# AlexandreDubray/consistent-viterbi

Measured on AMD Instinct MI355X. Metric: trellis cells/s (N*T*batch), N=256 T=512 batch=65536, higher is better.
Workload: dtype f64

## Files before the change

consistent-viterbi_amd/csrc/cviterbi.cpp:

```cpp
#include <hip/hip_runtime.h>

#include <algorithm>
#include <atomic>
#include <charconv>
#include <chrono>
#include <cmath>
#include <cstdarg>
#include <cstdio>
#include <cstdlib>
#include <cstring>
#include <memory>
#include <functional>
#include <limits>
#include <mutex>
#include <numeric>
#include <string>
#include <thread>
#include <type_traits>
#include <vector>

#include "../../include/cviterbi.h"
#include "batchplan.hpp"
#include "csp.hpp"
#include "hostscan.hpp"
// ... 60 lines not shown
    if (p) {
      (void)hipFree(p);
      g_dev_cur -= (int64_t)bytes;
    }
    p = nullptr;
    bytes = 0;
  }
  cv_status ensure(size_t n) {
    if (n <= bytes && p) return CV_OK;
    release();
    if (n == 0) n = 16;
    hipError_t e = hipMalloc(&p, n);
    if (e != hipSuccess) {
      p = nullptr;
      (void)hipGetLastError();
      return set_err(CV_ENOMEM, "hipMalloc(%zu) failed: %s", n, hipGetErrorString(e));
    }
    bytes = n;
    const int64_t cur = g_dev_cur += (int64_t)n;
    int64_t pk = g_dev_peak.load();
    while (cur > pk && !g_dev_peak.compare_exchange_weak(pk, cur)) {
    }
    return CV_OK;
  }
  template <typename T>
  T* as() const {
    return static_cast<T*>(p);
  }
};

cv_status upload(DevBuf& buf, const void* src, size_t bytes) {
  cv_status st = buf.ensure(bytes);
  if (st != CV_OK) return st;
  HIP_TRY(hipMemcpy(buf.p, src, bytes, hipMemcpyHostToDevice));
  return CV_OK;
}

constexpr uint64_t kDefaultWorkspace = 8ull << 30;
constexpr uint64_t kDefaultWorkspaceT64 = 64ull << 30;
constexpr size_t kMaxTimedEvents = 1 << 16;

}

struct PinnedHost {
  void* p = nullptr;
  size_t cap = 0;
  PinnedHost() = default;
  PinnedHost(const PinnedHost&) = delete;
  PinnedHost& operator=(const PinnedHost&) = delete;
  ~PinnedHost() { release(); }
  void release() {
    if (p) (void)hipHostFree(p);
    p = nullptr;
    cap = 0;
  }
  bool ensure(size_t bytes) {
    if (cap >= bytes && p) return true;
    if (p) (void)hipHostFree(p);
    p = nullptr;
    cap = 0;
    const size_t want = std::max<size_t>(bytes, 4096);
    if (hipHostMalloc(&p, want, hipHostMallocDefault) != hipSuccess) {
      (void)hipGetLastError();
      return false;
    }
    cap = want;
    return true;
  }
  template <typename T>
  T* as() const { return static_cast<T*>(p); }
};

struct OrderStage {
  int32_t* p[2] = {nullptr, nullptr};
  size_t cap[2] = {0, 0};
  hipEvent_t ev[2] = {nullptr, nullptr};
  bool pending[2] = {false, false};
  int slot = 0;
  OrderStage() = default;
  OrderStage(const OrderStage&) = delete;
  OrderStage& operator=(const OrderStage&) = delete;
  ~OrderStage() {
    for (int k = 0; k < 2; ++k) {
      if (pending[k]) (void)hipEventSynchronize(ev[k]);
      if (p[k]) (void)hipHostFree(p[k]);
      if (ev[k]) (void)hipEventDestroy(ev[k]);
    }
  }
  int32_t* acquire(size_t n) {
    const int k = slot;
    if (pending[k]) {
      if (hipEventSynchronize(ev[k]) != hipSuccess) return nullptr;
      pending[k] = false;
    }
    if (!ev[k] && hipEventCreateWithFlags(&ev[k], hipEventDisableTiming) != hipSuccess) return nullptr;
    if (cap[k] < n) {
      if (p[k]) (void)hipHostFree(p[k]);
      p[k] = nullptr;
      cap[k] = 0;
      const size_t want = std::max<size_t>(n, 4096);
      if (hipHostMalloc((void**)&p[k], want * 4, hipHostMallocDefault) != hipSuccess) return nullptr;
      cap[k] = want;
    }
    return p[k];
  }
  hipError_t release(hipStream_t stream) {
    const hipError_t e = hipEventRecord(ev[slot], stream);
    pending[slot] = e == hipSuccess;
    slot ^= 1;
    return e;
  }
};

struct cv_hmm {
  int N = 0, D = 0;
  std::vector<int64_t> bdims;
  int64_t V = 0;
  std::vector<double> pi, a, b;
  int device = 0;
  int cus = 0;
  hipStream_t stream = nullptr;
  hipStream_t bt_stream = nullptr;
  std::mutex mu;
  cvk::Tuning tuning;

  int np = 0;
  DevBuf t_aimg, t_pi, t_et, t_at, t_arm;
  int npw = 0;
  DevBuf w_arm, w_pi, w_et, w_at;
  DevBuf t_aimg_T, t_pi0;
  bool f64_ready = false;
  DevBuf d_pi64, d_a64, d_et64;
  DevBuf d_at64;

  int np64 = 0;
  bool t64_ready = false;
  DevBuf q_a, q_at, q_pi, q_et;
  DevBuf q_at32;
  bool t64_nonpos = false;
  int nonpos_cache = -1;
  double arc_max = -1.0;
  double cert_rho_cap = 0.0;
  DevBuf t64_stats;
  PinnedHost t64_stats_pin;
  bool t64_lo_off = false;
  int fx_state = -1;
  DevBuf fx_aimg, fx_pi, fx_et, fx_at;
  double fx_gain = 0.0;
  DevBuf fx_cert, fx_idx, fx_obs2, fx_path2, fx_score2, fx_status2;
  PinnedHost fx_cert_pin;
  std::vector<int64_t> fx_idx_host;
  bool fx_pinned = false;
  int64_t fx_last[4] = {0, 0, 0, 0};
  DevBuf q_pi0;
  bool g32_ready = false;
  DevBuf d_pi32, d_a32, d_et32;
  DevBuf d_at32;
  int pnp = 0;
  DevBuf p_pi, p_a, p_at, p_et, p_dump;
  DevBuf ps_rows, ps_order, st_gamma;
  DevBuf ps_kshift;
  PinnedHost sm_pin;
  OrderStage ps_pin;
  DevBuf kb_bp, kb_last, kb_order, kb_end, st_count;
  OrderStage kb_pin;
  DevBuf ws_main, ws_last, ws_order;
  struct SideWs {
    DevBuf main, last, order, idx, obs2, path2, res2;
    std::vector<int32_t> order_host;
    OrderStage order_pin;
    hipEvent_t ws_done = nullptr;
    bool ws_rec = false;
    std::vector<int64_t> idx_host;
    std::vector<hipEvent_t> ev;
    hipStream_t stream = nullptr;
    hipStream_t hi = nullptr;
    hipEvent_t start = nullptr, done = nullptr, after = nullptr;
  } side;
  DevBuf st_off, st_obs, st_path, st_score, st_status, st_forced;
  DevBuf st_emis;
  DevBuf cs_ranges, cs_delta, cs_g, cs_mu, cs_start, cs_zero, cs_queue;
  DevBuf cs_wrows;
  DevBuf cs_comp, cs_words;
  DevBuf cs_flag;
  DevBuf cs_seg;
  DevBuf rs_rows, rs_rowbase, rs_resume, rs_start, rs_off2, rs_ridx, rs_slot, rs_obs2, rs_frc2, rs_path2;
  DevBuf rs_srows, rs_srowbase, rs_cert;
  hipEvent_t rs_ev = nullptr;
  std::vector<int32_t> order_host;
  OrderStage order_pin;
  hipEvent_t ws_done = nullptr;
  bool ws_rec = false;
  std::vector<float> host_dl, host_mu;
  std::vector<int64_t> sort_pos;
  std::vector<hipEvent_t> ev;
  int64_t last_launches = 0;
  size_t last_ev_base = 0;
  bool acc_on = false, acc_overflow = false;
  size_t acc_used = 0;
  int32_t last_kernel = 0;
  int32_t last_np = 0;
  int32_t last_mt = -1;
  uint64_t last_explored = 0;
  int64_t last_traced = 0;
  int64_t last_chain[9] = {0, 0, 0, 0, 0, 0, 0, 0, 0};
  struct ChainBufs {
    DevBuf off, obs, path, res, cert, ebin, q, ends, gid, gpath;
    DevBuf first, rpsi, rows, small, rpath, soff, sobs, spath, sres, sinit, slast, spsi;
  } chainb;
  hipStream_t chain_stream = nullptr;
  std::vector<hipEvent_t> part_ev;
  std::vector<hipEvent_t> chunk_ev;
  std::vector<hipEvent_t> emis_ev;
  hipStream_t copy_stream = nullptr;
  PinnedHost chain_pin;
  PinnedHost chain_gpin;
  PinnedHost chain_obs_pin, chain_ring[2];
  hipEvent_t ring_ev[2] = {nullptr, nullptr};

  ~cv_hmm() {
    for (auto e : ring_ev)
      if (e) (void)hipEventDestroy(e);
    for (auto e : ev) (void)hipEventDestroy(e);
    for (auto e : side.ev) (void)hipEventDestroy(e);
    if (side.start) (void)hipEventDestroy(side.start);
    if (side.done) (void)hipEventDestroy(side.done);
    if (side.after) (void)hipEventDestroy(side.after);
    if (side.stream) (void)hipStreamDestroy(side.stream);
    if (side.hi) (void)hipStreamDestroy(side.hi);
    if (rs_ev) (void)hipEventDestroy(rs_ev);
    if (ws_done) (void)hipEventDestroy(ws_done);
    if (side.ws_done) (void)hipEventDestroy(side.ws_done);
    if (stream) (void)hipStreamDestroy(stream);
    if (bt_stream) (void)hipStreamDestroy(bt_stream);
    for (auto e : chunk_ev) (void)hipEventDestroy(e);
    for (auto e : emis_ev) (void)hipEventDestroy(e);
    for (auto e : part_ev) (void)hipEventDestroy(e);
    if (copy_stream) (void)hipStreamDestroy(copy_stream);
    if (chain_stream) (void)hipStreamDestroy(chain_stream);
  }
};

namespace {

uint64_t free_device_bytes(uint64_t held) {
  size_t fr = 0, tot = 0;
  if (hipMemGetInfo(&fr, &tot) != hipSuccess) {
    (void)hipGetLastError();
    return 0;
  }
  return (uint64_t)fr + held;
}

uint64_t default_workspace_cap(uint64_t held, uint64_t base) {
  const uint64_t avail = free_device_bytes(held);
  if (avail == 0) return base;
  return std::max<uint64_t>(std::min<uint64_t>(base, avail / 4 * 3), 256ull << 20);
}

cv_status set_device(cv_hmm* h) {
  int n = 0;
  if (hipGetDeviceCount(&n) != hipSuccess || n <= 0) {
    (void)hipGetLastError();
    return set_err(CV_EDEVICE, "no HIP device available");
  }
  if (h->device < 0 || h->device >= n) return set_err(CV_EDEVICE, "device %d out of range (%d devices)", h->device, n);
  HIP_TRY(hipSetDevice(h->device));
  if (!h->cus) HIP_TRY(hipDeviceGetAttribute(&h->cus, hipDeviceAttributeMultiprocessorCount, h->device));
  if (!h->stream) HIP_TRY(hipStreamCreateWithFlags(&h->stream, hipStreamNonBlocking));
  if (!h->bt_stream) HIP_TRY(hipStreamCreateWithFlags(&h->bt_stream, hipStreamNonBlocking));
  return CV_OK;
}

float f32(double x) { return (float)x; }

cv_status ensure_trellis_tables(cv_hmm* h) {
  const int np = cvk::trellis_padded_states(h->N);
  if (!np) return set_err(CV_EUNSUPPORTED, "trellis kernel covers 1 <= N <= 256 (N=%d)", h->N);
  if (h->np == np) return CV_OK;
  const int N = h->N;
  const int64_t V = h->V;
  const int R = np / 8;
  const float NI = -INFINITY;
  auto A = [&](int i, int j) -> float { return (i < N && j < N) ? f32(h->a[(size_t)i * N + j]) : NI; };
  std::vector<float> img((size_t)np * np);
  for (int w = 0; w < np / 16; ++w)
    for (int q = 0; q < R / 2; ++q)
      for (int lane = 0; lane < 64; ++lane) {
        const int rg = lane & 7, cp = lane >> 3, j0 = 16 * w + 2 * cp, r0 = rg * R + 2 * q;
        float* dst = &img[(((size_t)w * (R / 2) + q) * 64 + lane) * 4];
        dst[0] = A(r0, j0);
        dst[1] = A(r0, j0 + 1);
        dst[2] = A(r0 + 1, j0);
        dst[3] = A(r0 + 1, j0 + 1);
      }
  std::vector<float> pi(np, NI), at((size_t)np * np, NI), arm((size_t)np * np, NI), et((size_t)V * np, NI);
  for (int j = 0; j < N; ++j) pi[j] = f32(h->pi[j]);
  for (int i = 0; i < N; ++i)
    for (int j = 0; j < N; ++j) at[(size_t)j * np + i] = arm[(size_t)i * np + j] = f32(h->a[(size_t)i * N + j]);
  for (int j = 0; j < N; ++j)
    for (int64_t o = 0; o < V; ++o) et[(size_t)o * np + j] = f32(h->b[(size_t)j * V + o]);
  cv_status st;
  if ((st = upload(h->t_aimg, img.data(), img.size() * 4)) != CV_OK) return st;
  {
    auto AT = [&](int i, int j) -> float { return A(j, i); };
    std::vector<float> imgT((size_t)np * np);
// ... 1129 lines not shown
    if (err == hipSuccess) err = cvkb::launch_kbest_walk(g, stream);
    if (err != hipSuccess) return set_err(CV_EDEVICE, "K-best select / walk launch failed: %s", hipGetErrorString(err));
    HIP_TRY(hipEventRecord(b1, stream));
    h->last_launches = (int64_t)ci + 1;
  }
  return end_call(h, false, nev, stream);
}

cv_opts default_opts() {
  cv_opts o;
  cv_opts_init(&o);
  return o;
}

struct HostBatch {
  cv_hmm* h;
  int64_t nseq;
  const int64_t* offsets;
  const int32_t* obs;
  hipStream_t stream;
  int64_t base = 0, total = 0;
  hipError_t err = hipSuccess;

  size_t plane() const { return (size_t)std::max<int64_t>(total, 1); }

  cv_status stage(cv_opts& o, size_t planes, size_t width, bool check_obs = false, bool forced_host = true) {
    cv_status st = check_batch(nseq, offsets);
    if (st != CV_OK) return st;
    base = offsets[0], total = offsets[nseq];
    const int32_t* ob = check_obs ? obs : nullptr;
    const int32_t* fr = forced_host ? o.forced : nullptr;
    const int64_t V = h->V, N = h->N;
    int64_t k;
    if (ob && (k = first_bad(base, total, [&](int64_t i) { return ob[i] < 0 || ob[i] >= V; })) >= 0)
      return set_err(CV_EINVAL, "obs[%lld] = %d out of range [0,%lld)", (long long)k, ob[k], (long long)V);
    if (fr && (k = first_bad(base, total, [&](int64_t i) { return fr[i] < -1 || fr[i] >= N; })) >= 0)
      return set_err(CV_EINVAL, "forced[%lld] = %d out of range [-1,%d)", (long long)k, fr[k], h->N);
    if ((st = h->st_off.ensure((size_t)(nseq + 1) * 8)) != CV_OK) return st;
    if (obs && (st = h->st_obs.ensure(plane() * 4)) != CV_OK) return st;
    if (planes && (st = h->st_path.ensure(plane() * planes * 4)) != CV_OK) return st;
    if ((st = h->st_score.ensure((size_t)nseq * width * 8)) != CV_OK) return st;
    if ((st = h->st_status.ensure((size_t)nseq)) != CV_OK) return st;
    if (fr && (st = h->st_forced.ensure(plane() * 4)) != CV_OK) return st;
    HIP_TRY(hipMemcpyAsync(h->st_off.p, offsets, (size_t)(nseq + 1) * 8, hipMemcpyHostToDevice, stream));
    const size_t n = (size_t)(total - base) * 4;
    if (obs && n) HIP_TRY(hipMemcpyAsync(h->st_obs.as<int32_t>() + base, obs + base, n, hipMemcpyHostToDevice, stream));
    if (fr && n) HIP_TRY(hipMemcpyAsync(h->st_forced.as<int32_t>() + base, fr + base, n, hipMemcpyHostToDevice, stream));
    if (fr) o.forced = h->st_forced.as<int32_t>();
    return CV_OK;
  }
  cv_status stage_emis(const double* emis, int64_t ld, EmisSrc* src) {
    const int64_t N = h->N, rows = total - base;
    cv_status st = h->st_emis.ensure((size_t)std::max<int64_t>(rows, 1) * N * 8);
    if (st != CV_OK) return st;
    if (rows > 0)
      HIP_TRY(hipMemcpy2DAsync(h->st_emis.p, (size_t)N * 8, emis + base * ld, (size_t)ld * 8, (size_t)N * 8,
                               (size_t)rows, hipMemcpyHostToDevice, stream));
    *src = EmisSrc{reinterpret_cast<const double*>(reinterpret_cast<uintptr_t>(h->st_emis.p) -
                                                   (uintptr_t)base * (uintptr_t)N * 8),
                   N};
    return CV_OK;
  }
  cv_status fail(cv_status st) const {
    (void)hipStreamSynchronize(stream);
    return st;
  }
  template <typename T>
  void fetch_elems(T* out, const DevBuf& buf, size_t width = 1, size_t r = 0) {
    const size_t at = (r * (size_t)total + (size_t)base) * width, n = (size_t)(total - base) * width * sizeof(T);
    if (err == hipSuccess && n) err = hipMemcpyAsync(out + at, buf.as<T>() + at, n, hipMemcpyDeviceToHost, stream);
  }
  template <typename T>
  void fetch_seqs(T* out, const DevBuf& buf, size_t width = 1) {
    if (err == hipSuccess) err = hipMemcpyAsync(out, buf.p, (size_t)nseq * width * sizeof(T), hipMemcpyDeviceToHost, stream);
  }
  cv_status finish() {
    if (err == hipSuccess) err = hipStreamSynchronize(stream);
    return err == hipSuccess ? CV_OK : set_err(CV_EDEVICE, "copying the results back failed: %s", hipGetErrorString(err));
  }
};

}

extern "C" {

CV_API const char* cv_last_error(void) { return g_err.c_str(); }
CV_API const char* cv_version(void) { return "cviterbi 0.1.0 (gfx950)"; }
CV_API int32_t cv_abi_version(void) { return CV_ABI_VERSION; }
CV_API cv_status cv_device_memory(int64_t* current_bytes, int64_t* peak_bytes) {
  if (current_bytes) *current_bytes = g_dev_cur.load();
  if (peak_bytes) *peak_bytes = g_dev_peak.load();
  return CV_OK;
}
CV_API int32_t cv_device_count(void) {
  int n = 0;
  if (hipGetDeviceCount(&n) != hipSuccess) {
    (void)hipGetLastError();
    return 0;
  }
  return n;
}

CV_API void cv_opts_init(cv_opts* o) {
  if (!o) return;
  std::memset(o, 0, sizeof *o);
  o->dtype = CV_DTYPE_F64;
  o->assoc = CV_ASSOC_VITERBI;
  o->kernel = CV_KERNEL_AUTO;
  o->rescore_f64 = 1;
}

CV_API cv_status cv_hmm_create(const cv_hmm_desc* d, cv_hmm** out) {
  if (!d || !out) return set_err(CV_EINVAL, "null argument");
  if (d->ndims <= 0 || !d->bdims) return set_err(CV_EINVAL, "ndims/bdims required");
  std::vector<int64_t> bd(d->bdims, d->bdims + d->ndims);
  return make_hmm(d->nstates, bd, d->pi, d->a, d->b, d->device, out);
}

CV_API cv_status cv_hmm_from_json(const char* path, int32_t device, cv_hmm** out) {
  if (!path || !out) return set_err(CV_EINVAL, "null argument");
  std::string text, err;
  if (!cvh::read_file(path, text)) return set_err(CV_EIO, "cannot read %s", path);
  cvh::HmmJson j;
  if (!cvh::parse_hmm_json(text, j, err)) return set_err(CV_EPARSE, "%s", err.c_str());
  return make_hmm(j.nstates, j.bdims, j.pi.data(), j.a.data(), j.b.data(), device, out);
}

CV_API cv_status cv_hmm_write_json(const cv_hmm* h, const char* path) {
  if (!h || !path) return set_err(CV_EINVAL, "null argument");
  const std::string s = cvh::format_hmm_json(h->N, h->bdims, h->pi.data(), h->a.data(), h->b.data());
  FILE* f = fopen(path, "wb");
  if (!f) return set_err(CV_EIO, "cannot write %s", path);
  const size_t n = fwrite(s.data(), 1, s.size(), f);
  fclose(f);
  if (n != s.size()) return set_err(CV_EIO, "short write to %s", path);
  return CV_OK;
}

CV_API void cv_hmm_destroy(cv_hmm* h) {
  if (!h) return;
  int n = 0;
  if (hipGetDeviceCount(&n) == hipSuccess && h->device >= 0 && h->device < n) (void)hipSetDevice(h->device);
  delete h;
}

CV_API cv_status cv_hmm_set_tuning(cv_hmm* h, const char* key, int64_t value) {
  if (!h || !key) return set_err(CV_EINVAL, "bad argument");
  std::lock_guard<std::mutex> lk(h->mu);
  if (!cvk::tuning_set(h->tuning, key, value)) return set_err(CV_EINVAL, "unknown tuning key '%s' or value out of range", key);
  if (std::strcmp(key, "t64_nonpos") == 0) {
    h->nonpos_cache = -1;
    h->t64_ready = false;
    h->fx_state = -1;
  }
  return CV_OK;
}
CV_API cv_status cv_hmm_release_workspaces(cv_hmm* h) {
  if (!h) return set_err(CV_EINVAL, "null handle");
  CV_LOCK(h);
  cv_status st = set_device(h);
  if (st != CV_OK) return st;
  for (hipStream_t s : {h->stream, h->bt_stream, h->side.stream, h->side.hi, h->copy_stream, h->chain_stream})
    if (s) HIP_TRY(hipStreamSynchronize(s));
  if (h->ws_rec) HIP_TRY(hipEventSynchronize(h->ws_done));
  if (h->side.ws_rec) HIP_TRY(hipEventSynchronize(h->side.ws_done));
  for (DevBuf* b : {&h->ws_main, &h->ws_last, &h->ws_order, &h->side.main, &h->side.last, &h->side.order,
                    &h->side.idx, &h->side.obs2, &h->side.path2, &h->side.res2, &h->st_off, &h->st_obs, &h->st_path,
                    &h->st_score, &h->st_status, &h->st_forced, &h->cs_ranges, &h->cs_delta, &h->cs_g, &h->cs_mu,
                    &h->cs_start, &h->cs_zero, &h->cs_queue, &h->cs_wrows, &h->cs_comp, &h->cs_words, &h->cs_flag,
                    &h->cs_seg, &h->rs_rows, &h->rs_rowbase, &h->rs_resume, &h->rs_start, &h->rs_off2, &h->rs_ridx,
                    &h->rs_slot, &h->rs_obs2, &h->rs_frc2, &h->rs_path2, &h->rs_srows, &h->rs_srowbase, &h->rs_cert,
                    &h->chainb.off, &h->chainb.obs, &h->chainb.path, &h->chainb.res, &h->chainb.cert, &h->chainb.ebin,
                    &h->chainb.q, &h->chainb.ends, &h->chainb.gid, &h->chainb.gpath, &h->chainb.first,
                    &h->chainb.rpsi, &h->chainb.rows, &h->chainb.small, &h->chainb.rpath, &h->chainb.soff,
                    &h->chainb.sobs, &h->chainb.spath, &h->chainb.sres, &h->chainb.sinit, &h->chainb.slast,
                    &h->chainb.spsi, &h->ps_rows,
                    &h->ps_order, &h->ps_kshift, &h->st_gamma, &h->kb_bp, &h->kb_last, &h->kb_order, &h->kb_end, &h->st_count,
                    &h->st_emis, &h->fx_cert, &h->fx_idx, &h->fx_obs2, &h->fx_path2, &h->fx_score2, &h->fx_status2})
    b->release();
  h->fx_cert_pin.release();
  h->sm_pin.release();
  h->ws_rec = false;
  h->side.ws_rec = false;
  h->chain_pin.release();
  h->chain_gpin.release();
  h->chain_obs_pin.release();
  h->chain_ring[0].release();
  h->chain_ring[1].release();
  return CV_OK;
}
CV_API cv_status cv_hmm_get_tuning(const cv_hmm* h, const char* key, int64_t* value) {
  if (!h || !key || !value) return set_err(CV_EINVAL, "bad argument");
  std::lock_guard<std::mutex> lk(const_cast<cv_hmm*>(h)->mu);
  if (!cvk::tuning_get(h->tuning, key, value)) return set_err(CV_EINVAL, "unknown tuning key '%s'", key);
  return CV_OK;
}
CV_API const char* cv_tuning_key(int32_t i) { return cvk::tuning_key(i); }
CV_API int32_t cv_hmm_nstates(const cv_hmm* h) { return h ? h->N : -1; }
CV_API int64_t cv_hmm_nobs(const cv_hmm* h) { return h ? h->V : -1; }
CV_API int32_t cv_hmm_ndims(const cv_hmm* h) { return h ? h->D : -1; }
CV_API cv_status cv_hmm_bdims(const cv_hmm* h, int64_t* out) {
  if (!h || !out) return set_err(CV_EINVAL, "null argument");
  std::copy(h->bdims.begin(), h->bdims.end(), out);
  return CV_OK;
}

CV_API cv_status cv_obs_flatten(const cv_hmm* h, const int64_t* value, int64_t* flat) {
  if (!h || !value || !flat) return set_err(CV_EINVAL, "null argument");
  int64_t f = 0;
  for (int d = 0; d < h->D; ++d) {
    if (value[d] < 0 || value[d] >= h->bdims[d])
      return set_err(CV_EINVAL, "observation component %d = %lld out of range [0,%lld)", d, (long long)value[d],
                     (long long)h->bdims[d]);
    f = f * h->bdims[d] + value[d];
  }
  *flat = f;
  return CV_OK;
}

static bool lookup_ok(const cv_hmm* h, int32_t s, int64_t o) {
  return h && s >= 0 && s < h->N && o >= 0 && o < h->V;
}

CV_API double cv_hmm_init_prob(const cv_hmm* h, int32_t state, int64_t obs) {
  if (!lookup_ok(h, state, obs)) return NAN;
  return h->pi[state] + h->b[(size_t)state * h->V + obs];
}
CV_API cv_status cv_hmm_init_probs(const cv_hmm* h, int64_t obs, double* out) {
  if (!lookup_ok(h, 0, obs) || !out) return set_err(CV_EINVAL, "bad argument");
  for (int s = 0; s < h->N; ++s) out[s] = h->pi[s] + h->b[(size_t)s * h->V + obs];
  return CV_OK;
}
CV_API double cv_hmm_transition_prob(const cv_hmm* h, int32_t from, int32_t to, int64_t obs) {
  if (!lookup_ok(h, to, obs) || from < 0 || from >= h->N) return NAN;
  return h->a[(size_t)from * h->N + to] + h->b[(size_t)to * h->V + obs];
}
CV_API cv_status cv_hmm_transitions_to(const cv_hmm* h, int32_t to, double* out) {
  if (!h || to < 0 || to >= h->N || !out) return set_err(CV_EINVAL, "bad argument");
  for (int s = 0; s < h->N; ++s) out[s] = h->a[(size_t)s * h->N + to];
  return CV_OK;
}
CV_API double cv_hmm_emit_prob(const cv_hmm* h, int32_t state, int64_t obs) {
  if (!lookup_ok(h, state, obs)) return NAN;
  return h->b[(size_t)state * h->V + obs];
}
CV_API cv_status cv_hmm_emit_probs(const cv_hmm* h, int64_t obs, double* out) {
  if (!lookup_ok(h, 0, obs) || !out) return set_err(CV_EINVAL, "bad argument");
  for (int s = 0; s < h->N; ++s) out[s] = h->b[(size_t)s * h->V + obs];
  return CV_OK;
}

static int32_t fix_quantise(double x) {
  const double r = std::nearbyint(std::ldexp(x, -cvk::kFixQLog2));
  return r > (double)cvk::kFixFloor ? (int32_t)r : cvk::kFixFloor;
}

static cv_status ensure_fix_tables(cv_hmm* h) {
  if (h->fx_state >= 0) return CV_OK;
  const int np = cvk::trellis_padded_states(h->N);
  if (!cvk::fix_supported(np) || !model_nonpos(h)) {
    h->fx_state = 0;
    return CV_OK;
  }
  const int N = h->N;
  const int64_t V = h->V;
  const int R = np / 8;
  const int32_t F = cvk::kFixFloor;
  auto A = [&](int i, int j) -> int32_t { return (i < N && j < N) ? fix_quantise(h->a[(size_t)i * N + j]) : F; };
  std::vector<int32_t> img((size_t)np * np), pi((size_t)np, F), at((size_t)np * np, F), et((size_t)V * np, F);
  for (int w = 0; w < np / 16; ++w)
    for (int q = 0; q < R / 2; ++q)
      for (int lane = 0; lane < 64; ++lane) {
        const int rg = lane & 7, cp = lane >> 3, j0 = 16 * w + 2 * cp, r0 = rg * R + 2 * q;
        int32_t* dst = &img[(((size_t)w * (R / 2) + q) * 64 + lane) * 4];
        dst[0] = A(r0, j0);
        dst[1] = A(r0, j0 + 1);
        dst[2] = A(r0 + 1, j0);
        dst[3] = A(r0 + 1, j0 + 1);
      }
  for (int j = 0; j < N; ++j) pi[(size_t)j] = fix_quantise(h->pi[(size_t)j]);
  for (int i = 0; i < N; ++i)
    for (int j = 0; j < N; ++j) at[(size_t)j * np + i] = A(i, j);
  parallel_ranges(N, [&](int, int64_t lo, int64_t hi) {
    for (int64_t j = lo; j < hi; ++j)
      for (int64_t o = 0; o < V; ++o) et[(size_t)o * np + j] = fix_quantise(h->b[(size_t)j * V + o]);
  }, std::max<int64_t>(1, 4096 / std::max<int64_t>(V, 1)));
  double wmax = 0.0;
  for (const std::vector<double>* v : {&h->pi, &h->a, &h->b}) {
    double m = 0.0;
    for (double x : *v)
      if (std::isfinite(x)) m = std::max(m, std::fabs(x));
    wmax += m;
  }
  h->fx_gain = 1.01 * 2.02 * std::ldexp(1.0, -53 - cvk::kFixQLog2) * wmax;
  cv_status st;
  if ((st = upload(h->fx_aimg, img.data(), img.size() * 4)) != CV_OK) return st;
  if ((st = upload(h->fx_pi, pi.data(), pi.size() * 4)) != CV_OK) return st;
  if ((st = upload(h->fx_at, at.data(), at.size() * 4)) != CV_OK) return st;
  if ((st = upload(h->fx_et, et.data(), et.size() * 4)) != CV_OK) return st;
  h->fx_state = 1;
  return CV_OK;
}

static cv_status fixed_first_decode(cv_hmm* h, int64_t nseq, const int64_t* offsets_host, const int64_t* offsets_dev,
                                    const int32_t* obs_dev, const cv_opts& o, int32_t* path_dev, double* score_dev,
                                    uint8_t* status_dev, hipStream_t stream, bool* done) {
  *done = false;
  h->fx_last[0] = h->fx_last[1] = h->fx_last[2] = 0;
  h->fx_last[3] = h->fx_pinned ? 1 : 0;
  const int64_t min_elems = h->tuning.t64_fixed_first;
  if (min_elems <= 0 || h->fx_pinned || h->fx_state == 0 || nseq < 2 || nseq > INT32_MAX) return CV_OK;
  if (o.dtype != CV_DTYPE_F64 || o.assoc != CV_ASSOC_VITERBI || o.forced || o.flags != 0 ||
      (o.kernel != CV_KERNEL_AUTO && o.kernel != CV_KERNEL_TRELLIS_F64))
    return CV_OK;
  std::vector<int64_t> off_copy;
  cv_status st = host_offsets(nseq, offsets_host, offsets_dev, off_copy, stream);
  if (st != CV_OK) return st;
  if (offsets_host[nseq] - offsets_host[0] < min_elems) return CV_OK;
  if ((st = ensure_fix_tables(h)) != CV_OK) return st;
  if (h->fx_state != 1) return CV_OK;
  if ((st = ensure_f64_tables(h)) != CV_OK) return st;
  const int np = cvk::trellis_padded_states(h->N);

  const uint64_t per_elem = (uint64_t)np * 4;
  const uint64_t cap = o.workspace_bytes ? o.workspace_bytes : default_workspace_cap(h->ws_main.bytes, kDefaultWorkspaceT64);
  const int fchunks = h->tuning.t64_fixed_chunks;
  const bool one_stream = fchunks <= 0;
  std::vector<cvplan::Chunk> chunks;
  cvplan::split_pipelined(offsets_host, nseq,
                          {per_elem, cap, one_stream, one_stream ? 8u : (uint64_t)std::min(fchunks, 64),
                           2 * (int64_t)std::max(h->cus, 1)},
                          chunks);
  const cvplan::Shares largest = cvplan::measure(offsets_host, chunks);
  const bool serial = one_stream || chunks.size() == 1;
  const int nbuf = serial ? 1 : 2;
  const size_t buf_bytes = ((std::max<uint64_t>(largest.max_elems, 1) * per_elem + 255) / 256) * 256;
  if ((st = h->ws_main.ensure(buf_bytes * nbuf)) != CV_OK) return st;
  if ((st = h->fx_cert.ensure((size_t)nseq)) != CV_OK) return st;
  if (!h->fx_cert_pin.ensure((size_t)nseq)) return set_err(CV_ENOMEM, "pinned certificate copy failed");
  if (h->ws_rec) HIP_TRY(hipStreamWaitEvent(stream, h->ws_done, 0));
  const bool varlen = cvplan::varlen(offsets_host, nseq);
  std::vector<int64_t> npair(chunks.size(), 0);
  const int32_t* order_dev = nullptr;
  if (varlen) {
    h->order_host.resize((size_t)nseq);
    cvplan::longest_first(offsets_host, chunks, h->order_host.data(), npair.data(), h->sort_pos);
    if ((st = upload_order(h->ws_order, h->order_pin, h->order_host.data(), nseq, stream, &order_dev)) != CV_OK) return st;
  }
  HIP_TRY(hipMemsetAsync(h->fx_cert.p, 0, (size_t)nseq, stream));

  const bool acc_was = h->acc_on;
  const size_t acc_base = acc_was ? h->acc_used : 0;
  if (!acc_was) h->acc_on = true, h->acc_used = 0;
  struct AccRestore {
    cv_hmm* h;
    bool was;
    ~AccRestore() {
      if (!was) h->acc_on = false, h->acc_used = 0;
    }
  } acc_restore{h, acc_was};
  const size_t nev = 4 * chunks.size();
  size_t eb;
  if ((st = reserve_events(h, false, nev, &eb)) != CV_OK) return st;
  hipStream_t bts = serial ? stream : h->bt_stream;
  struct BtJoin {
    hipStream_t s;
    bool pending = false;
    ~BtJoin() {
      if (pending) (void)hipStreamSynchronize(s);
    }
  } bt_join{h->bt_stream};
  for (size_t ci = 0; ci < chunks.size(); ++ci) {
    const cvplan::Chunk c = chunks[ci];
    const int64_t n = c.second - c.first;
    const int64_t np2 = varlen ? npair[ci] : n / 2;
    hipEvent_t* const e4 = &h->ev[eb + 4 * ci];
    hipEvent_t f0 = e4[0], f1 = e4[1], b0 = e4[2], b1 = e4[3];
    if (!serial && ci >= 2) HIP_TRY(hipStreamWaitEvent(stream, h->ev[eb + 4 * (ci - 2) + 3], 0));
    HIP_TRY(hipEventRecord(f0, stream));
    cvk::FixFwdArgs fa{};
    fa.a_img = h->fx_aimg.as<int32_t>();
    fa.pi = h->fx_pi.as<int32_t>();
    fa.et = h->fx_et.as<int32_t>();
    fa.offsets = offsets_dev;
    fa.obs = obs_dev;
    fa.order = order_dev;
    fa.seq_begin = c.first;
    fa.rows = reinterpret_cast<int32_t*>(h->ws_main.as<unsigned char>() + (nbuf == 2 ? ci % 2 : 0) * buf_bytes);
    fa.row_elem_base = offsets_host[c.first];
    fa.cert = h->fx_cert.as<uint8_t>();
    fa.nobs = (int)h->V;
    hipError_t err = cvk::launch_fix_fwd2(np, fa, np2, stream);
    if (err != hipSuccess) return set_err(CV_EDEVICE, "fixed-point forward launch failed: %s", hipGetErrorString(err));
    HIP_TRY(hipEventRecord(f1, stream));
    if (!serial) {
      HIP_TRY(hipStreamWaitEvent(bts, f1, 0));
      bt_join.pending = true;
    }
    HIP_TRY(hipEventRecord(b0, bts));
    const int reserve = (serial || ci + 1 == chunks.size()) ? 0 : 100 * 1024;
    cvk::FixBtArgs ba{};
    ba.rows = fa.rows;
    ba.row_elem_base = fa.row_elem_base;
    ba.at = h->fx_at.as<int32_t>();
    ba.offsets = offsets_dev;
    ba.order = order_dev;
    ba.seq_begin = c.first;
    ba.seq_end = c.first + 2 * np2;
    ba.gain = h->fx_gain;
    ba.path = path_dev;
    ba.cert = fa.cert;
    err = cvk::launch_fix_bt(np, ba, bts, reserve);
    if (err == hipSuccess) {
      cvk::FixScoreArgs ra{};
      ra.path = path_dev;
      ra.obs = obs_dev;
      ra.offsets = offsets_dev;
      ra.seq_begin = c.first;
      ra.seq_end = c.second;
      ra.nstates = h->N;
      ra.pi64 = h->d_pi64.as<double>();
      ra.a64 = h->d_a64.as<double>();
      ra.et64 = h->d_et64.as<double>();
      ra.cert = fa.cert;
      ra.score = score_dev;
      ra.status = status_dev;
      err = cvk::launch_fix_score(ra, bts, reserve);
    }
    if (err != hipSuccess) return set_err(CV_EDEVICE, "fixed-point backtrack launch failed: %s", hipGetErrorString(err));
    HIP_TRY(hipEventRecord(b1, bts));
  }
  if (!serial) {
    HIP_TRY(hipStreamWaitEvent(stream, h->ev[eb + 4 * (chunks.size() - 1) + 3], 0));
    bt_join.pending = false;
  }
  if ((st = end_call(h, false, nev, stream)) != CV_OK) return st;
  HIP_TRY(hipMemcpyAsync(h->fx_cert_pin.p, h->fx_cert.p, (size_t)nseq, hipMemcpyDeviceToHost, stream));
  HIP_TRY(hipStreamSynchronize(stream));

  const uint8_t* cert = h->fx_cert_pin.as<uint8_t>();
  std::vector<int64_t>& ix = h->fx_idx_host;
  int64_t nfb = 0, nfail = 0;
  for (int64_t s = 0; s < nseq; ++s) nfb += cert[s] != 1, nfail += cert[s] == 2;
  h->fx_last[0] = 1;
  h->fx_last[1] = nseq - nfb;
  h->fx_last[2] = nfb;
  h->fx_last[3] = 0;
  if (nfail * 8 > nseq - nfb + nfail) {
    h->fx_pinned = true;
    h->fx_last[1] = 0, h->fx_last[2] = nseq, h->fx_last[3] = 1;
    if (acc_was) h->acc_used = acc_base;
    return CV_OK;
  }
  *done = true;
  h->last_kernel = CV_KERNEL_TRELLIS_F64;
  h->last_np = np;
  h->last_mt = 2;
  if (nfb > 0) {
    ix.resize((size_t)(3 * nfb + 1));
    int64_t *cstart = ix.data(), *off2 = cstart + nfb, *perm = off2 + nfb + 1;
    int64_t k = 0;
    off2[0] = 0;
    for (int64_t s = 0; s < nseq; ++s)
      if (cert[s] != 1) {
        cstart[k] = offsets_host[s];
        off2[k + 1] = off2[k] + (offsets_host[s + 1] - offsets_host[s]);
        perm[k++] = s;
      }
    const int64_t elems2 = off2[nfb];
    if ((st = h->fx_idx.ensure(ix.size() * 8)) != CV_OK) return st;
    if ((st = h->fx_obs2.ensure((size_t)std::max<int64_t>(elems2, 1) * 4)) != CV_OK) return st;
    if ((st = h->fx_path2.ensure((size_t)std::max<int64_t>(elems2, 1) * 4)) != CV_OK) return st;
    if ((st = h->fx_score2.ensure((size_t)nfb * 8)) != CV_OK) return st;
    if ((st = h->fx_status2.ensure((size_t)nfb)) != CV_OK) return st;
    HIP_TRY(hipMemcpyAsync(h->fx_idx.p, ix.data(), ix.size() * 8, hipMemcpyHostToDevice, stream));
    const int64_t *d_cstart = h->fx_idx.as<int64_t>(), *d_off2 = d_cstart + nfb, *d_perm = d_off2 + nfb + 1;
    hipError_t err = cvk::launch_compact_suffix(d_cstart, d_off2, obs_dev, nullptr, nullptr, h->fx_obs2.as<int32_t>(),
                                                nullptr, nfb, stream);
    if (err != hipSuccess) return set_err(CV_EDEVICE, "fallback gather launch failed: %s", hipGetErrorString(err));
    DecodeReq rq;
    rq.batch_api = true;
    if ((st = decode_device(h, nfb, off2, d_off2, h->fx_obs2.as<int32_t>(), o, h->fx_path2.as<int32_t>(),
                            h->fx_score2.as<double>(), h->fx_status2.as<uint8_t>(), stream, rq)) != CV_OK)
      return st;
    err = cvk::launch_scatter_suffix(d_cstart, d_off2, d_perm, h->fx_path2.as<int32_t>(), h->fx_score2.as<double>(),
                                     h->fx_status2.as<uint8_t>(), path_dev, score_dev, status_dev, nfb, stream);
    if (err != hipSuccess) return set_err(CV_EDEVICE, "fallback scatter launch failed: %s", hipGetErrorString(err));
    if ((st = end_call(h, false, 0, stream)) != CV_OK) return st;
  }
  h->last_ev_base = acc_base;
  h->last_launches = (int64_t)((h->acc_used - acc_base) / 4);
  return CV_OK;
}

CV_API cv_status cv_decode_batch_device(cv_hmm* h, int64_t nseq, const int64_t* offsets_host,
                                        const int64_t* offsets_dev, const int32_t* obs_dev, const cv_opts* opts,
                                        int32_t* path_dev, double* score_dev, uint8_t* status_dev) {
  if (!h) return set_err(CV_EINVAL, "null handle");
  if (nseq > 0 && (!offsets_dev || !obs_dev || !path_dev || !score_dev || !status_dev))
    return set_err(CV_EINVAL, "null device buffer");
  CV_LOCK(h);
  cv_status st = set_device(h);
  if (st != CV_OK) return st;
  const cv_opts o = opts ? *opts : default_opts();
  hipStream_t stream = o.stream ? (hipStream_t)o.stream : h->stream;
  bool done = false;
  st = fixed_first_decode(h, nseq, offsets_host, offsets_dev, obs_dev, o, path_dev, score_dev, status_dev, stream, &done);
  if (st != CV_OK || done) return st;
  DecodeReq rq;
  rq.batch_api = true;
  return decode_device(h, nseq, offsets_host, offsets_dev, obs_dev, o, path_dev, score_dev, status_dev, stream, rq);
}

static cv_status decode_host_locked(cv_hmm* h, int64_t nseq, const int64_t* offsets, const int32_t* obs, cv_opts o,
                                    int32_t* path_out, double* score_out, uint8_t* status_out,
                                    bool obs_staged = false, bool forced_staged = false, bool batch_api = false) {
  cv_status st;
  if (nseq == 0) return CV_OK;
  HostBatch hb{h, nseq, offsets, obs_staged ? nullptr : obs, o.stream ? (hipStream_t)o.stream : h->stream};
  if ((st = hb.stage(o, 1, 1, true, !forced_staged)) != CV_OK) return st;
  DecodeReq rq;
  rq.batch_api = batch_api;
  bool done = false;
  if (batch_api && !forced_staged)
    st = fixed_first_decode(h, nseq, offsets, h->st_off.as<int64_t>(), h->st_obs.as<int32_t>(), o,
                            h->st_path.as<int32_t>(), h->st_score.as<double>(), h->st_status.as<uint8_t>(), hb.stream,
                            &done);
  if (st == CV_OK && !done)
    st = decode_device(h, nseq, offsets, h->st_off.as<int64_t>(), h->st_obs.as<int32_t>(), o, h->st_path.as<int32_t>(),
                       h->st_score.as<double>(), h->st_status.as<uint8_t>(), hb.stream, rq);
  if (st != CV_OK) return hb.fail(st);
  hb.fetch_elems(path_out, h->st_path);
  hb.fetch_seqs(score_out, h->st_score);
  hb.fetch_seqs(status_out, h->st_status);
  return hb.finish();
}

CV_API cv_status cv_decode_batch(cv_hmm* h, int64_t nseq, const int64_t* offsets, const int32_t* obs,
                                 const cv_opts* opts, int32_t* path_out, double* score_out, uint8_t* status_out) {
  if (!h) return set_err(CV_EINVAL, "null handle");
  if (nseq < 0 || (nseq > 0 && (!offsets || !obs || !path_out || !score_out || !status_out)))
    return set_err(CV_EINVAL, "null argument");
  CV_LOCK(h);
  cv_status st = set_device(h);
  if (st != CV_OK) return st;
  return decode_host_locked(h, nseq, offsets, obs, opts ? *opts : default_opts(), path_out, score_out, status_out,
                            false, false, true);
}

CV_API cv_status cv_posterior_batch_device(cv_hmm* h, int64_t nseq, const int64_t* offsets_host,
                                           const int64_t* offsets_dev, const int32_t* obs_dev, const cv_opts* opts,
                                           double* loglik_dev, int32_t* path_dev, double* gamma_dev,
                                           uint8_t* status_dev) {
  if (!h) return set_err(CV_EINVAL, "null handle");
  if (nseq < 0) return set_err(CV_EINVAL, "nseq < 0");
  if (nseq > 0 && (!offsets_dev || !obs_dev || !loglik_dev || !status_dev))
    return set_err(CV_EINVAL, "null device buffer");
  CV_LOCK(h);
  cv_status st = set_device(h);
  if (st != CV_OK) return st;
  const cv_opts o = opts ? *opts : default_opts();
  hipStream_t stream = o.stream ? (hipStream_t)o.stream : h->stream;
  return posterior_device(h, nseq, offsets_host, offsets_dev, obs_dev, o, loglik_dev, path_dev, gamma_dev, status_dev,
                          stream);
}

CV_API cv_status cv_posterior_batch(cv_hmm* h, int64_t nseq, const int64_t* offsets, const int32_t* obs,
                                    const cv_opts* opts, double* loglik_out, int32_t* path_out, double* gamma_out,
                                    uint8_t* status_out) {
  if (!h) return set_err(CV_EINVAL, "null handle");
  if (nseq < 0 || (nseq > 0 && (!offsets || !obs || !loglik_out || !status_out)))
    return set_err(CV_EINVAL, "null argument");
  CV_LOCK(h);
  cv_status st = set_device(h);
  if (st != CV_OK) return st;
  cv_opts o = opts ? *opts : default_opts();
  if (nseq == 0) return CV_OK;
  const size_t N = (size_t)h->N;
  HostBatch hb{h, nseq, offsets, obs, o.stream ? (hipStream_t)o.stream : h->stream};
  if ((st = hb.stage(o, path_out ? 1 : 0, 1)) != CV_OK) return st;
  if (gamma_out && (st = h->st_gamma.ensure(hb.plane() * N * 8)) != CV_OK) return st;
  st = posterior_device(h, nseq, offsets, h->st_off.as<int64_t>(), h->st_obs.as<int32_t>(), o, h->st_score.as<double>(),
                        path_out ? h->st_path.as<int32_t>() : nullptr, gamma_out ? h->st_gamma.as<double>() : nullptr,
                        h->st_status.as<uint8_t>(), hb.stream);
  if (st != CV_OK) return hb.fail(st);
  if (path_out) hb.fetch_elems(path_out, h->st_path);
  if (gamma_out) hb.fetch_elems(gamma_out, h->st_gamma, N);
  hb.fetch_seqs(loglik_out, h->st_score);
  hb.fetch_seqs(status_out, h->st_status);
  if ((st = hb.finish()) != CV_OK) return st;
  for (int64_t s = 0; s < nseq; ++s)
    if (status_out[s] == CV_SEQ_INFEASIBLE)
      return set_err(CV_EINFEASIBLE, "sequence %lld has likelihood 0", (long long)s);
  return CV_OK;
}

CV_API cv_status cv_sample_batch_device(cv_hmm* h, int64_t nseq, const int64_t* offsets_host,
// ... 1331 lines not shown
  if (first_bad_obs != ~0ull)
    return set_err(CV_EINVAL, "obs[%llu] out of range [0,%lld)", first_bad_obs, (long long)h->V);
  trace_mark("device constrained: checks + constrained list");
  SideJoin side{h};
  const bool side_off = h->tuning.no_side != 0;
  if (!side_off && o.dtype == CV_DTYPE_F64 && resume_supported(h, true) && !cs.empty()) {
    if ((st = side_streams(h)) != CV_OK) return st;
    HIP_TRY(hipEventRecord(h->side.start, stream));
    HIP_TRY(hipStreamWaitEvent(h->side.hi, h->side.start, 0));
    stream = h->side.hi;
    o.stream = stream;
    side.hi = true;
  }
  auto launch_side = [&]() -> cv_status {
    return side.hi ? side_decode_launch(h, nseq, offsets_host, obs_dev, cs, o, path_dev, score_dev, status_dev, stream,
                                        &side.active)
                   : CV_OK;
  };
  const std::vector<int32_t> pairs = conseq_pairs(cs, component);
  const int64_t npairs = (int64_t)pairs.size() / 2;
  std::vector<int64_t> part((size_t)cvcsp::partial_words((int)h->N, ncomp, npairs), 0);
  PrefixKeep keep;
  if ((st = constrained_partials_locked(h, nseq, offsets_host, nullptr, component, ncomp, pairs.data(), npairs, o,
                                        part.data(), &cs, nullptr, obs_dev, &keep, launch_side)) != CV_OK)
    return st;
  uint64_t explored = 0;
  if ((st = select_locked((int32_t)h->N, ncomp, pairs.data(), npairs, part.data(), comp_state_out, &explored)) !=
      CV_OK)
    return st;
  h->last_explored = explored;
  trace_mark("select");
  if (keep.kept) {
    if ((st = forced_decode_resume(h, nseq, offsets_host, offsets_dev, obs_dev, component, comp_state_out, cs, keep,
                                   o, path_dev, score_dev, status_dev, stream, side.active)) != CV_OK)
      return st;
  } else {
    if (side.active) HIP_TRY(hipStreamWaitEvent(stream, h->side.done, 0));
    if ((st = stage_forced_locked(h, offsets_host, nseq, component, comp_state_out, cs, stream)) != CV_OK) return st;
    o.forced = h->st_forced.as<int32_t>();
    if ((st = decode_device(h, nseq, offsets_host, offsets_dev, obs_dev, o, path_dev, score_dev, status_dev,
                            stream)) != CV_OK) {
      (void)hipStreamSynchronize(stream);
      return st;
    }
  }
  if (side.active) {
    HIP_TRY(hipStreamWaitEvent(stream, h->side.done, 0));
    side.active = false;
  }
  std::vector<double> sc((size_t)nseq);
  std::vector<uint8_t> ss((size_t)nseq);
  HIP_TRY(hipMemcpyAsync(sc.data(), score_dev, (size_t)nseq * 8, hipMemcpyDeviceToHost, stream));
  HIP_TRY(hipMemcpyAsync(ss.data(), status_dev, (size_t)nseq, hipMemcpyDeviceToHost, stream));
  HIP_TRY(hipStreamSynchronize(stream));
  const double obj = mark_unassigned(nseq, component, comp_state_out, cs, sc.data(), ss.data());
  if (objective_out) *objective_out = obj;
  bool fixed = false;
  for (const auto& c : cs)
    for (int64_t e : c.elems) fixed |= comp_state_out[component[e]] < 0;
  if (fixed) {
    HIP_TRY(hipMemcpyAsync(score_dev, sc.data(), (size_t)nseq * 8, hipMemcpyHostToDevice, stream));
    HIP_TRY(hipMemcpyAsync(status_dev, ss.data(), (size_t)nseq, hipMemcpyHostToDevice, stream));
    HIP_TRY(hipStreamSynchronize(stream));
  }
  trace_mark("forced decode (device)");
  return CV_OK;
}

CV_API cv_status cv_decode_constrained_exchange(cv_hmm* h, int64_t nseq, const int64_t* offsets, const int32_t* obs,
                                                const int32_t* component, int32_t ncomp, int64_t npairs,
                                                const int32_t* pairs, cv_exchange_fn exchange, void* ctx,
                                                const cv_opts* opts, int32_t* path_out, double* score_out,
                                                uint8_t* status_out, int32_t* comp_state_out,
                                                uint64_t* explored_out, double* objective_out) {
  if (!h) return set_err(CV_EINVAL, "null handle");
  if (nseq < 0 || ncomp < 0 || npairs < 0 ||
      (nseq > 0 && (!offsets || !obs || !component || !path_out || !score_out || !status_out)) ||
      (ncomp > 0 && !comp_state_out) || (npairs > 0 && !pairs))
    return set_err(CV_EINVAL, "null argument");
  if (!pairs_sorted(pairs, npairs, ncomp)) return set_err(CV_EINVAL, "pairs must be sorted (c1 < c2) and unique");
  CV_LOCK(h);
  cv_status st = set_device(h);
  if (st != CV_OK) return st;
  cv_opts o = opts ? *opts : default_opts();
  for (int32_t c = 0; c < ncomp; ++c) comp_state_out[c] = -1;
  if (objective_out) *objective_out = 0.0;
  if (explored_out) *explored_out = 0;
  std::vector<ConSeq> cs;
  if (nseq > 0 && (st = constrained_validate(h, nseq, offsets, obs, component, ncomp, o, cs)) != CV_OK) return st;
  std::vector<int64_t> part((size_t)std::max<int64_t>(cvcsp::partial_words((int)h->N, ncomp, npairs), 1), 0);
  bool obs_staged = false;
  PrefixKeep keep;
  if (nseq > 0 && (st = constrained_partials_locked(h, nseq, offsets, obs, component, ncomp, pairs, npairs, o,
                                                    part.data(), &cs, &obs_staged, nullptr, &keep)) != CV_OK)
    return st;
  trace_mark("exchange: shard partials");
  if (exchange && exchange(part.data(), cvcsp::partial_words((int)h->N, ncomp, npairs), ctx) != 0)
    return set_err(CV_EDEVICE, "exchange callback failed");
  trace_mark("exchange: callback");
  uint64_t explored = 0;
  if ((st = select_locked((int32_t)h->N, ncomp, pairs, npairs, part.data(), comp_state_out, &explored)) != CV_OK)
    return st;
  h->last_explored = explored;
  if (explored_out) *explored_out = explored;
  if (nseq == 0) return CV_OK;
  return final_decode_host(h, nseq, offsets, obs, component, comp_state_out, o, cs, keep, obs_staged, path_out,
                           score_out, status_out, objective_out);
}

namespace {
cv_status sum_timing(cv_hmm* h, size_t eb, int64_t launches, cv_timing* out) {
  if (launches == 0) return CV_OK;
  HIP_TRY(hipSetDevice(h->device));
  const int64_t L = launches;
  HIP_TRY(hipEventSynchronize(h->ev[eb + 4 * (L - 1) + 3]));
  for (int64_t c = 0; c < L; ++c) {
    float f = 0, b = 0;
    HIP_TRY(hipEventElapsedTime(&f, h->ev[eb + 4 * c], h->ev[eb + 4 * c + 1]));
    HIP_TRY(hipEventElapsedTime(&b, h->ev[eb + 4 * c + 2], h->ev[eb + 4 * c + 3]));
    out->fwd_ms += f;
    out->bt_ms += b;
  }
  float tot = 0;
  HIP_TRY(hipEventElapsedTime(&tot, h->ev[eb], h->ev[eb + 4 * (L - 1) + 3]));
  out->total_ms = tot;
  return CV_OK;
}
}

CV_API cv_status cv_last_superseq_stats(const cv_hmm* h, int64_t* out) {
  if (!h || !out) return set_err(CV_EINVAL, "null argument");
  for (int q = 0; q < 9; ++q) out[q] = h->last_chain[q];
  return CV_OK;
}

CV_API int32_t cv_last_t64_stats(const cv_hmm* h, int64_t* out, int32_t n) {
  if (!h || n < 0 || (n > 0 && !out)) {
    set_err(CV_EINVAL, "bad argument");
    return -1;
  }
  int64_t v[8];
  t64_stats_sum(h, v);
  for (int32_t q = 0; q < n && q < 8; ++q) out[q] = v[q];
  return 8;
}

CV_API int32_t cv_last_fixed_first_stats(const cv_hmm* h, int64_t* out, int32_t n) {
  if (!h || n < 0 || (n > 0 && !out)) {
    set_err(CV_EINVAL, "bad argument");
    return -1;
  }
  for (int32_t q = 0; q < n && q < 4; ++q) out[q] = h->fx_last[q];
  return 4;
}

CV_API cv_status cv_last_suffix_traced(const cv_hmm* h, int64_t* out) {
  if (!h || !out) return set_err(CV_EINVAL, "null argument");
  *out = h->last_traced;
  return CV_OK;
}

CV_API cv_status cv_last_timing(cv_hmm* h, cv_timing* out) {
  if (!h || !out) return set_err(CV_EINVAL, "null argument");
  CV_LOCK(h);
  std::memset(out, 0, sizeof *out);
  out->launches = h->last_launches;
  out->kernel = h->last_kernel;
  out->padded_states = h->last_np;
  out->mfma_tiles = h->last_mt;
  return sum_timing(h, h->last_ev_base, h->last_launches, out);
}

CV_API cv_status cv_timing_begin(cv_hmm* h) {
  if (!h) return set_err(CV_EINVAL, "null argument");
  CV_LOCK(h);
  h->acc_on = true;
  h->acc_overflow = false;
  h->acc_used = 0;
  return CV_OK;
}

CV_API cv_status cv_timing_end(cv_hmm* h, cv_timing* out) {
  if (!h || !out) return set_err(CV_EINVAL, "null argument");
  CV_LOCK(h);
  std::memset(out, 0, sizeof *out);
  const bool was_on = h->acc_on, overflow = h->acc_overflow;
  const size_t used = h->acc_used;
  h->acc_on = false;
  h->acc_overflow = false;
  h->acc_used = 0;
  if (!was_on && !overflow) return set_err(CV_EINVAL, "cv_timing_end without cv_timing_begin");
  if (overflow) return set_err(CV_ELIMIT, "more than %zu chunk launches timed since cv_timing_begin", kMaxTimedEvents / 4);
  out->launches = (int64_t)(used / 4);
  out->kernel = h->last_kernel;
  out->padded_states = h->last_np;
  out->mfma_tiles = h->last_mt;
  return sum_timing(h, 0, out->launches, out);
}

CV_API cv_status cv_viterbi_decode(cv_hmm* h, int64_t T, const int32_t* obs, int32_t* path_out) {
  if (!h || T < 0 || (T > 0 && (!obs || !path_out))) return set_err(CV_EINVAL, "bad argument");
  if (T == 0) return CV_OK;
  const int64_t off[2] = {0, T};
  double score;
  uint8_t status;
  cv_opts o;
  cv_opts_init(&o);
  o.dtype = CV_DTYPE_F64;
  o.assoc = CV_ASSOC_DECODE;
  o.rescore_f64 = 0;
  return cv_decode_batch(h, 1, off, obs, &o, path_out, &score, &status);
}

}

namespace {
cv_status chain_backtrack(int NP, const uint16_t* psi, int64_t L, int32_t end_state, int32_t* path_dev,
                          hipStream_t stream) {
  const int64_t seg = std::max<int64_t>(256, (L + 8191) / 8192);
  const int64_t nseg = (L + seg - 1) / seg;
  DevBuf d_map, d_end;
  cv_status st;
  if ((st = d_map.ensure((size_t)nseg * NP * 2)) != CV_OK) return st;
  if ((st = d_end.ensure((size_t)nseg * 4)) != CV_OK) return st;
  cvk::CpChainBtArgs b{};
  b.psi = psi;
  b.np = NP;
  b.len = L;
  b.seg = seg;
  b.nseg = nseg;
  b.map = d_map.as<uint16_t>();
  b.end_state = d_end.as<int32_t>();
  b.path = path_dev;
  hipError_t err = cvk::launch_cp_chain_seg_map(b, stream);
  if (err != hipSuccess) return set_err(CV_EDEVICE, "chain backtrack (maps) failed: %s", hipGetErrorString(err));
  std::vector<uint16_t> map((size_t)nseg * NP);
  if (nseg > 1) {
    HIP_TRY(hipMemcpyAsync(map.data(), d_map.p, map.size() * 2, hipMemcpyDeviceToHost, stream));
    HIP_TRY(hipStreamSynchronize(stream));
  }
  std::vector<int32_t> end((size_t)nseg);
  int32_t s = end_state;
  for (int64_t k = nseg - 1; k >= 0; --k) {
    end[(size_t)k] = s;
    if (k > 0) s = map[(size_t)k * NP + s];
  }
  HIP_TRY(hipMemcpyAsync(d_end.p, end.data(), (size_t)nseg * 4, hipMemcpyHostToDevice, stream));
  err = cvk::launch_cp_chain_seg_path(b, stream);
  if (err != hipSuccess) return set_err(CV_EDEVICE, "chain backtrack (paths) failed: %s", hipGetErrorString(err));
  HIP_TRY(hipStreamSynchronize(stream));
  return CV_OK;
}

cv_status superseq_cp_wg(cv_hmm* h, int64_t L, const int32_t* obs, const std::vector<uint8_t>& first,
                         int32_t* path_out, double* objective_out) {
  cv_status st;
  if ((st = ensure_t64_tables(h)) != CV_OK) return st;
  const int NP = h->np64;
  const uint64_t psi_bytes = (uint64_t)L * NP * 2;
  const uint64_t avail = free_device_bytes(0);
  if (avail && psi_bytes + (uint64_t)L * 9 > avail / 10 * 9)
    return set_err(CV_ENOMEM,
                   "super-sequence of %lld elements needs %.1f GB of back-pointers (%.1f GB of device memory "
                   "free): decode it in parts or per sequence (solver kind gpu-cp-seq)",
                   (long long)L, psi_bytes / 1e9, avail / 1e9);
  hipStream_t stream = h->stream;
  DevBuf d_obs, d_first, d_psi, d_path, d_out;
  if ((st = d_obs.ensure((size_t)L * 4)) != CV_OK) return st;
  if ((st = d_first.ensure((size_t)L)) != CV_OK) return st;
  if ((st = d_psi.ensure((size_t)psi_bytes)) != CV_OK) return st;
  if ((st = d_path.ensure((size_t)L * 4)) != CV_OK) return st;
  if ((st = d_out.ensure(16)) != CV_OK) return st;
  HIP_TRY(hipMemcpyAsync(d_obs.p, obs, (size_t)L * 4, hipMemcpyHostToDevice, stream));
  HIP_TRY(hipMemcpyAsync(d_first.p, first.data(), (size_t)L, hipMemcpyHostToDevice, stream));
  cvk::CpChainWgArgs g{};
  g.pi = h->q_pi.as<double>();
  g.a = h->q_a.as<double>();
  g.et = h->q_et.as<double>();
  g.obs = d_obs.as<int32_t>();
  g.first = d_first.as<uint8_t>();
  g.len = L;
  g.nstates = h->N;
  g.psi = d_psi.as<uint16_t>();
  g.objective = d_out.as<double>();
  g.final_state = reinterpret_cast<int32_t*>(d_out.as<double>() + 1);
  hipError_t err = cvk::launch_cp_chain_wg(NP, g, stream);
  if (err != hipSuccess) return set_err(CV_EDEVICE, "super-sequence chain launch failed: %s", hipGetErrorString(err));
  double out[2];
  HIP_TRY(hipMemcpyAsync(out, d_out.p, 16, hipMemcpyDeviceToHost, stream));
  HIP_TRY(hipStreamSynchronize(stream));
  *objective_out = out[0];
  int32_t fs;
  std::memcpy(&fs, &out[1], 4);
  if ((st = chain_backtrack(NP, d_psi.as<uint16_t>(), L, fs, d_path.as<int32_t>(), stream)) != CV_OK) return st;
  HIP_TRY(hipMemcpyAsync(path_out, d_path.p, (size_t)L * 4, hipMemcpyDeviceToHost, stream));
  HIP_TRY(hipStreamSynchronize(stream));
  if (!(*objective_out > -INFINITY))
    return set_err(CV_EINFEASIBLE, "no finite-probability path through the super-sequence (cp.rs:87 asserts)");
  return CV_OK;
}


cv_status superseq_cp_par(cv_hmm* h, int64_t nseq, const int64_t* offsets, const int32_t* obs, int32_t* path_out,
                          double* objective_out, bool* applied) {
  *applied = false;
  cv_status st;
// ... 1464 lines not shown
```

consistent-viterbi_amd/csrc/kernels/trellis.h:

```cpp
#pragma once
#include <hip/hip_runtime.h>
#include <stdint.h>

namespace cvk {

enum { CVK_SEQ_OK = 0, CVK_SEQ_INFEASIBLE = 1, CVK_SEQ_EMPTY = 2, CVK_SEQ_BADOBS = 3 };
enum { CVK_ASSOC_VITERBI = 0, CVK_ASSOC_CP = 1, CVK_ASSOC_DP = 2, CVK_ASSOC_DECODE = 3 };

struct TrellisFwdArgs {
  const float* a_img;
  const float* pi;
  const float* et;
  const int64_t* offsets;
  const int32_t* obs;
  const int32_t* order;
  int64_t seq_begin;
  float* delta;
  int64_t delta_elem_base;
  uint8_t* status;
  int nobs;
  const int32_t* forced;
  const int64_t* ranges;
  int reverse;
  float* last_row;
  const int32_t* start;
  int64_t split;
  const float* a_img2;
  const float* pi2;
  float* last_row2;
  const int32_t* slot_order;
  const int64_t* row_base;
  const float* resume_rows;
};

struct BacktrackArgs {
  const float* delta;
  int64_t delta_elem_base;
  const float* at;
  const int64_t* offsets;
  const int32_t* obs;
  const int32_t* order;
  int64_t seq_begin, seq_end;
  int nstates;
  int32_t* path;
  double* score;
  float* score32;
  uint8_t* status;
};

struct RescoreArgs {
  const int32_t* path;
  const int32_t* obs;
  const int64_t* offsets;
  const int32_t* order;
  int64_t seq_begin, seq_end;
  int nstates;
  const double* pi64;
  const double* a64;
  const double* et64;
  const uint8_t* status;
  double* score;
};
hipError_t launch_rescore_f64(const RescoreArgs& r, int64_t nseq, hipStream_t stream, int lds_reserve = 0);

constexpr int kFixQLog2 = -26;
constexpr int32_t kFixFloor = -(1 << 30);
struct FixFwdArgs {
  const int32_t* a_img;
  const int32_t* pi;
  const int32_t* et;
  const int64_t* offsets;
  const int32_t* obs;
  const int32_t* order;
  int64_t seq_begin;
  int32_t* rows;
  int64_t row_elem_base;
  uint8_t* cert;
  int nobs;
};
struct FixBtArgs {
  const int32_t* rows;
  int64_t row_elem_base;
  const int32_t* at;
  const int64_t* offsets;
  const int32_t* order;
  int64_t seq_begin, seq_end;
  double gain;
  int32_t* path;
  uint8_t* cert;
};
struct FixScoreArgs {
  const int32_t* path;
  const int32_t* obs;
  const int64_t* offsets;
  int64_t seq_begin, seq_end;
  int nstates;
  const double* pi64;
  const double* a64;
  const double* et64;
  uint8_t* cert;
  double* score;
  uint8_t* status;
};
bool fix_supported(int np);
hipError_t launch_fix_fwd2(int np, const FixFwdArgs& fa, int64_t npairs, hipStream_t stream);
hipError_t launch_fix_bt(int np, const FixBtArgs& ba, hipStream_t stream, int lds_reserve = 0);
hipError_t launch_fix_score(const FixScoreArgs& r, hipStream_t stream, int lds_reserve = 0);

template <typename REAL>
struct GenericFwdArgs {
  const int32_t* forced;
  const REAL* a;
  const REAL* pi;
  const REAL* et;
  const int64_t* offsets;
  const int32_t* obs;
  const int32_t* order;
  int64_t seq_begin;
  int nstates, nobs, assoc;
  uint16_t* psi;
  int64_t psi_elem_base;
  REAL* last_row;
  uint8_t* status;
  REAL* rows;
  const REAL* cp_init;
  REAL* cp_last;
  REAL* grows;
  int64_t wide_steps;
  int prio;
};

template <typename REAL>
struct GenericBtArgs {
  const uint16_t* psi;
  int64_t psi_elem_base;
  const REAL* last_row;
  const int64_t* offsets;
  const int32_t* order;
  int64_t seq_begin, seq_end;
  int nstates;
  int32_t* path;
  double* score;
  uint8_t* status;
  const int32_t* obs;
  int rescore_f64;
  int decode_bt;
  const double* pi64;
  const double* a64;
  const double* et64;
  const REAL* rows;
  const REAL* at;
  const REAL* et;
  int assoc, nobs;
};

struct MaxMarginalArgs {
  const float* delta;
  const float* g;
  const int64_t* ranges_suffix;
  const float* at;
  float* mu;
};
hipError_t launch_max_marginal(int np, const MaxMarginalArgs& a, int64_t ncon, hipStream_t stream);

hipError_t launch_scatter_forced(const int64_t* elems, const int32_t* states, int64_t n, int32_t* forced,
                                 hipStream_t stream);

hipError_t launch_obs_first_bad(const int32_t* obs, int64_t lo, int64_t hi, int64_t V, unsigned long long* first,
                                hipStream_t stream);

hipError_t launch_resume_rows(const float* last, const int32_t* state, int64_t n, int np, float* out,
                              hipStream_t stream);
hipError_t launch_compact_suffix(const int64_t* cstart, const int64_t* off2, const int32_t* obs, const int32_t* forced,
                                 const int32_t* ridx, int32_t* obs2, int32_t* forced2, int64_t nseq,
                                 hipStream_t stream);
hipError_t launch_scatter_suffix(const int64_t* cstart, const int64_t* off2, const int64_t* perm,
                                 const int32_t* path2, const double* score2, const uint8_t* status2, int32_t* path,
                                 double* score, uint8_t* status, int64_t nseq, hipStream_t stream);
struct PrefixBtArgs {
  const float* rows;
  const int64_t* row_base;
  const int64_t* seq;
  const int64_t* t1;
  const int32_t* state;
  const int64_t* offsets;
  const float* at;
  const uint8_t* status;
  int32_t* path;
};
hipError_t launch_prefix_backtrack(int np, const PrefixBtArgs& a, int64_t n, hipStream_t stream, int lds_reserve);
hipError_t launch_zero_infeasible_prefix(const PrefixBtArgs& a, int64_t n, hipStream_t stream);

int trellis_padded_states(int n);
hipError_t launch_trellis_fwd(int np, const TrellisFwdArgs& fa, int64_t nseq, hipStream_t stream);
bool trellis_pair_supported(int np);
hipError_t launch_trellis_fwd2(int np, const TrellisFwdArgs& fa, int64_t npairs, hipStream_t stream);
hipError_t launch_trellis_bt(int np, const BacktrackArgs& ba, int64_t nseq, hipStream_t stream, int lds_reserve = 0);
int trellis_wave_states(int n);
hipError_t launch_trellis_wave(int npw, const TrellisFwdArgs& fa, const BacktrackArgs& ba, int64_t nseq,
                               hipStream_t stream);
template <typename REAL>
hipError_t launch_generic_fwd(const GenericFwdArgs<REAL>& fa, int64_t nseq, hipStream_t stream);
template <typename REAL>
hipError_t launch_generic_bt(const GenericBtArgs<REAL>& ba, int64_t nseq, hipStream_t stream);
template <typename REAL>
hipError_t launch_generic_bt_rows(const GenericBtArgs<REAL>& ba, int64_t nseq, hipStream_t stream);
int generic_max_states(int real_bytes);
constexpr int kGenericGlobalMaxStates = 65535;
bool generic_wide(int n, int real_bytes, int64_t nseq, bool cp);

struct GenericExtArgs {
  const double* tab;
  const double* pi;
  const double* et;
  const int32_t* obs;
  const int64_t* ranges;
  const int32_t* start;
  int reverse, noemit_last;
  int nstates;
  double* last_row;
  double* grows;
  int64_t wide_steps;
};
hipError_t launch_generic_ext(const GenericExtArgs& g, int64_t nslots, hipStream_t stream);
bool generic_ext_wide(int n);

}
```

consistent-viterbi_amd/csrc/kernels/trellis.hip:

```cpp
#include <hip/hip_runtime.h>
#include <stdint.h>
#include <stdlib.h>

#include <algorithm>

#include "trellis.h"
#include "../tuning.h"

namespace cvk {

__device__ __forceinline__ float ninf_f() { return -__builtin_inff(); }

__device__ __forceinline__ float octet_max(float x) {
  asm volatile(
      "s_nop 1\n\t"
      "v_max_f32_dpp %0, %0, %0 quad_perm:[1,0,3,2] row_mask:0xf bank_mask:0xf\n\t"
      "s_nop 1\n\t"
      "v_max_f32_dpp %0, %0, %0 quad_perm:[2,3,0,1] row_mask:0xf bank_mask:0xf\n\t"
      "s_nop 1\n\t"
      "v_max_f32_dpp %0, %0, %0 row_half_mirror row_mask:0xf bank_mask:0xf"
      : "+v"(x));
  return x;
}

// ... 896 lines not shown
    ldst[lds_w] = dn;
    (drow + (size_t)t * NP)[jw] = dn;
    post_max(dn, &mus[t % 3]);
    if (first) {
      lds_barrier();
      ld8(nsrc, P);
    }
  };
  auto step = [&](int t) {
    const int cur = (t - 1) & 1, nxt = t & 1;
    half(&lds[0][cur][rg * S], &lds[1][cur][rg * S], &lds[0][nxt][0], dX, mu[0], t, eXr, eYr, oY, true, clampT(t + 1));
    half(&lds[1][cur][rg * S], &lds[0][nxt][rg * S], &lds[1][nxt][0], dY, mu[1], t, eYr, eXr, oX, false, clampT(t + 2));
  };
  for (int t = 1; t < T; ++t) step(t);
  if (bad && lane == 0 && w == 0) {
    if (bad & 1u) args.cert[seqX] = CVK_SEQ_BADOBS;
    if (bad & 2u) args.cert[seqY] = CVK_SEQ_BADOBS;
  }
}

template <int NP>
__global__ __launch_bounds__(256) void backtrack_fix_i32(FixBtArgs args) {
  constexpr int VL = NP / 64;
  constexpr int PF = 8;
  constexpr int F = kFixFloor;
  static_assert(VL == 4, "int4 rows");
  const int lane = threadIdx.x & 63;
  const int64_t slot = args.seq_begin + (int64_t)blockIdx.x * 4 + (threadIdx.x >> 6);
  if (slot >= args.seq_end) return;
  const int64_t seq = args.order ? (int64_t)args.order[slot] : slot;
  const int64_t e0 = args.offsets[seq];
  const int T = (int)(args.offsets[seq + 1] - e0);
  if (T <= 0 || args.cert[seq] != 0) return;
  int32_t* __restrict__ path = args.path + e0;
  const int32_t* __restrict__ drow = args.rows + (e0 - args.row_elem_base) * NP + VL * lane;
  const int32_t* __restrict__ at = args.at + VL * lane;
  const double g = args.gain;
  auto extra = [&](int n) { return (long long)fmin(floor(g * (double)n * (double)n), 536870912.0); };
  auto load_row = [&](int r, int (&dst)[VL]) {
    if (r >= 0) {
      const int4 x = *reinterpret_cast<const int4*>(drow + (size_t)r * NP);
      dst[0] = x.x, dst[1] = x.y, dst[2] = x.z, dst[3] = x.w;
    } else {
      dst[0] = dst[1] = dst[2] = dst[3] = F;
    }
  };
  auto top2 = [&](const int (&s)[VL], int& M, int& M2) -> int {
    M = wave_max_i(max(max(s[0], s[1]), max(s[2], s[3])));
    int fk = VL;
#pragma unroll
    for (int k = VL - 1; k >= 0; --k) fk = (s[k] == M) ? k : fk;
    const unsigned long long mask = __ballot(fk < VL);
    const int L = (int)__builtin_ctzll(mask);
    const int win = VL * L + __builtin_amdgcn_readlane(fk, L);
    int o = INT32_MIN;
#pragma unroll
    for (int k = 0; k < VL; ++k) o = max(o, (VL * lane + k == win) ? INT32_MIN : s[k]);
    M2 = wave_max_i(o);
    return win;
  };
  auto fail = [&] {
    if (lane == 0) args.cert[seq] = 2;
  };
  int cur, M, M2;
  {
    int last[VL];
    load_row(T - 1, last);
    cur = top2(last, M, M2);
    if (!(M > F && (long long)M - M2 >= 2ll * T + 1 + extra(T + 1))) return fail();
  }
  int pathreg = 0;
  if (lane == ((T - 1) & 63)) pathreg = cur;
  if (((T - 1) & 63) == 0 && lane == 0) path[T - 1] = cur;
  int ring[PF][VL];
#pragma unroll
  for (int u = 0; u < PF; ++u) load_row(T - 2 - u, ring[u]);
  for (int base = T - 1; base >= 1; base -= PF) {
#pragma unroll
    for (int u = 0; u < PF; ++u) {
      const int t = base - u;
      if (t >= 1) {
        const int4 ac = *reinterpret_cast<const int4*>(at + (size_t)cur * NP);
        const int sv[VL] = {ring[u][0] + ac.x, ring[u][1] + ac.y, ring[u][2] + ac.z, ring[u][3] + ac.w};
        cur = top2(sv, M, M2);
        if (!(M > F && (long long)M - M2 >= 2ll * t + 2 + extra(t + 1))) return fail();
        const int tp = t - 1;
        if (lane == (tp & 63)) pathreg = cur;
        if ((tp & 63) == 0 && tp + lane < T) path[tp + lane] = pathreg;
      }
    }
#pragma unroll
    for (int u = 0; u < PF; ++u) load_row(base - PF - 1 - u, ring[u]);
  }
  if (lane == 0) args.cert[seq] = 1;
}

__global__ __launch_bounds__(64) void fix_score_f64(FixScoreArgs r) {
  const int64_t seq = r.seq_begin + (int64_t)blockIdx.x * 64 + threadIdx.x;
  if (seq >= r.seq_end || r.cert[seq] != 1) return;
  const int64_t e0 = r.offsets[seq];
  const int T = (int)(r.offsets[seq + 1] - e0);
  const int32_t* __restrict__ path = r.path + e0;
  const int32_t* __restrict__ obs = r.obs + e0;
  const int N = r.nstates;
  auto kept = [](double x) { return __builtin_rint(x * 67108864.0) > (double)kFixFloor; };
  static_assert(kFixQLog2 == -26, "kept() scales by 2^26");
  int pp = path[0];
  const double p0 = r.pi64[pp], b0 = r.et64[(size_t)obs[0] * N + pp];
  bool ok = kept(p0) && kept(b0);
  double d = p0 + b0;
  for (int t = 1; t < T; ++t) {
    const int p = path[t];
    const double bv = r.et64[(size_t)obs[t] * N + p];
    ok = ok && kept(bv);
    d = (d + r.a64[(size_t)pp * N + p]) + bv;
    pp = p;
  }
  if (ok) {
    r.score[seq] = d;
    r.status[seq] = CVK_SEQ_OK;
  } else {
    r.cert[seq] = 2;
  }
}

bool fix_supported(int np) { return np == 256; }

hipError_t launch_fix_fwd2(int np, const FixFwdArgs& fa, int64_t npairs, hipStream_t stream) {
  if (npairs <= 0) return hipSuccess;
  if (np != 256) return hipErrorInvalidValue;
  hipLaunchKernelGGL((trellis_fwd2_i32<256>), dim3((unsigned)npairs), dim3(1024), 0, stream, fa);
  return hipGetLastError();
}

hipError_t launch_fix_bt(int np, const FixBtArgs& ba, hipStream_t stream, int lds_reserve) {
  const int64_t n = ba.seq_end - ba.seq_begin;
  if (n <= 0) return hipSuccess;
  if (np != 256) return hipErrorInvalidValue;
  if (lds_reserve > 0)
    (void)hipFuncSetAttribute(reinterpret_cast<const void*>(&backtrack_fix_i32<256>),
                              hipFuncAttributeMaxDynamicSharedMemorySize, 160 * 1024);
  hipLaunchKernelGGL((backtrack_fix_i32<256>), dim3((unsigned)((n + 3) / 4)), dim3(256), (size_t)lds_reserve, stream,
                     ba);
  return hipGetLastError();
}

hipError_t launch_fix_score(const FixScoreArgs& r, hipStream_t stream, int lds_reserve) {
  const int64_t n = r.seq_end - r.seq_begin;
  if (n <= 0) return hipSuccess;
  if (lds_reserve > 0)
    (void)hipFuncSetAttribute(reinterpret_cast<const void*>(&fix_score_f64), hipFuncAttributeMaxDynamicSharedMemorySize,
                              160 * 1024);
  hipLaunchKernelGGL(fix_score_f64, dim3((unsigned)((n + 63) / 64)), dim3(64), (size_t)lds_reserve, stream, r);
  return hipGetLastError();
}

template <int NPW, bool FRC>
__global__ __launch_bounds__(256) void trellis_wave_f32(TrellisFwdArgs args, BacktrackArgs bargs) {
  constexpr int C = NPW / 16;
  constexpr int R = NPW / 4;
  constexpr int LS = R + 4;
  static_assert(NPW % 16 == 0 && NPW >= 16 && NPW <= 64, "NPW in {16, 32, 48, 64}");
  __shared__ __attribute__((aligned(16))) float lds_all[4][2][4 * LS];
  __shared__ __attribute__((aligned(16))) float at_lds[NPW * NPW];
  for (int k = threadIdx.x; k < NPW * NPW; k += 256) at_lds[k] = bargs.at[k];
  __syncthreads();
  const int lane = threadIdx.x & 63;
  const int wv = __builtin_amdgcn_readfirstlane(threadIdx.x >> 6);
  const int rg = lane & 3, cq = lane >> 2;
  const int p = rg & 1, q = rg >> 1;
  const int jw = C == 4 ? 4 * cq + 2 * p + q : C == 3 ? 3 * cq + (q ? 2 : p) : C == 2 ? 2 * cq + p : cq;
  const int64_t slot = args.seq_begin + 4 * (int64_t)blockIdx.x + wv;
  if (slot >= bargs.seq_end) return;
  int64_t seq, e0;
  int T;
  seq_range<false>(args, slot, seq, e0, T);
  if (T <= 0) {
    if (lane == 0) {
      bargs.score[seq] = 0.0;
      bargs.status[seq] = CVK_SEQ_EMPTY;
    }
    return;
  }
  float(*lds)[4 * LS] = lds_all[wv];
  typedef const __attribute__((address_space(4))) int32_t* cobs_t;
  const cobs_t obs = (cobs_t)(args.obs + e0);
  const cobs_t frc = (cobs_t)(FRC ? args.forced + e0 : nullptr);
  float* __restrict__ drow = args.delta + (e0 - args.delta_elem_base) * NPW;
  const unsigned V = (unsigned)args.nobs;
  float a_reg[R * C];
  if constexpr (C == 4) {
    const float4* src = reinterpret_cast<const float4*>(args.a_img) + (size_t)(R * rg) * (NPW / 4) + cq;
#pragma unroll
    for (int r = 0; r < R; ++r) {
      const float4 v = src[r * (NPW / 4)];
      a_reg[4 * r + 0] = v.x;
      a_reg[4 * r + 1] = v.y;
      a_reg[4 * r + 2] = v.z;
      a_reg[4 * r + 3] = v.w;
    }
  } else {
    const float* src = args.a_img + (size_t)(R * rg) * NPW + C * cq;
#pragma unroll
    for (int r = 0; r < R; ++r)
#pragma unroll
      for (int k = 0; k < C; ++k) a_reg[C * r + k] = src[(size_t)r * NPW + k];
  }
  unsigned bad = 0;
  auto obs_s = [&](int t) -> unsigned {
    const unsigned o = (unsigned)obs[t];
    bad |= (o >= V);
    return o < V ? o : 0u;
  };
  auto force = [&](float d, int f) -> float { return (FRC && f >= 0 && jw != f) ? ninf_f() : d; };
  const int wofs = (jw / R) * LS + (jw % R);
  {
    const float d0 = force(args.pi[jw] + args.et[(size_t)obs_s(0) * NPW + jw], FRC ? frc[0] : -1);
    lds[0][wofs] = d0;
    drow[jw] = d0;
  }
  const int Tm1 = T - 1;
  unsigned so[4];
  float pe[4];
#pragma unroll
  for (int k = 0; k < 4; ++k) {
    pe[k] = args.et[(size_t)obs_s(min(1 + k, Tm1)) * NPW + jw];
    so[k] = obs_s(min(5 + k, Tm1));
  }
  for (int t0 = 1; t0 < T; t0 += 4) {
#pragma unroll
    for (int k = 0; k < 4; ++k) {
      const int t = t0 + k;
      if (t >= T) break;
      const int f_use = FRC ? frc[t] : -1;
      const float* src = &lds[(t - 1) & 1][rg * LS];
      float4 d[R / 4];
#pragma unroll
      for (int b = 0; b < R / 4; ++b) d[b] = *reinterpret_cast<const float4*>(src + 4 * b);
      float c[C];
#pragma unroll
      for (int kc = 0; kc < C; ++kc) {
        float m = fmaxf(d[0].x + a_reg[0 * C + kc], d[0].y + a_reg[1 * C + kc]);
        m = fmaxf(fmaxf(m, d[0].z + a_reg[2 * C + kc]), d[0].w + a_reg[3 * C + kc]);
#pragma unroll
        for (int b = 1; b < R / 4; ++b) {
          m = fmaxf(fmaxf(m, d[b].x + a_reg[(4 * b + 0) * C + kc]), d[b].y + a_reg[(4 * b + 1) * C + kc]);
          m = fmaxf(fmaxf(m, d[b].z + a_reg[(4 * b + 2) * C + kc]), d[b].w + a_reg[(4 * b + 3) * C + kc]);
        }
        c[kc] = m;
      }
      float kk;
      if constexpr (C == 4) {
        float k0 = p ? c[2] : c[0], k1 = p ? c[3] : c[1];
        const float g0 = p ? c[0] : c[2], g1 = p ? c[1] : c[3];
        k0 = dpp_max_xor1_other(k0, g0);
        k1 = dpp_max_xor1_other(k1, g1);
        kk = q ? k1 : k0;
        const float gg = q ? k0 : k1;
        kk = dpp_max_xor2_other(kk, gg);
      } else if constexpr (C == 3) {
        float k0 = p ? c[1] : c[0];
        const float g0 = p ? c[0] : c[1];
        k0 = dpp_max_xor1_other(k0, g0);
        const float k2 = dpp_max_xor1(c[2]);
        kk = q ? k2 : k0;
        const float gg = q ? k0 : k2;
        kk = dpp_max_xor2_other(kk, gg);
      } else if constexpr (C == 2) {
        float k0 = p ? c[1] : c[0];
        const float g0 = p ? c[0] : c[1];
        k0 = dpp_max_xor1_other(k0, g0);
        kk = dpp_max_xor2(k0);
      } else {
        kk = dpp_max_xor2(dpp_max_xor1(c[0]));
      }
#ifndef CVK_ABLATE_NOEMIT
      const float e_use = pe[k];
#else
      const float e_use = -0.5f * (float)(t & 7);
#endif
      const float dn = force(kk + e_use, f_use);
      lds[t & 1][wofs] = dn;
      drow[(size_t)t * NPW + jw] = dn;
#ifndef CVK_ABLATE_NOEMIT
      pe[k] = args.et[(size_t)so[k] * NPW + jw];
      so[k] = obs_s(min(t + 8, Tm1));
#endif
    }
  }
  __builtin_amdgcn_fence(__ATOMIC_RELEASE, "agent");
  __builtin_amdgcn_fence(__ATOMIC_ACQUIRE, "agent");
#ifndef CVK_ABLATE_NOBT
  backtrack_one<1, NPW>(bargs, seq, e0, T, lane, drow + lane, at_lds + lane, bad != 0);
#endif
}

__global__ __launch_bounds__(64) void rescore_f64_lanes(RescoreArgs r) {
  const int64_t slot = r.seq_begin + (int64_t)blockIdx.x * 64 + threadIdx.x;
  if (slot >= r.seq_end) return;
  const int64_t seq = r.order ? (int64_t)r.order[slot] : slot;
  if (r.status[seq] != CVK_SEQ_OK) return;
  const int64_t e0 = r.offsets[seq];
  const int T = (int)(r.offsets[seq + 1] - e0);
  const int32_t* __restrict__ path = r.path + e0;
  const int32_t* __restrict__ obs = r.obs + e0;
  const int N = r.nstates;
// ... 1269 lines not shown
```

consistent-viterbi_amd/csrc/tuning.cpp:

```cpp
#include "tuning.h"

#include <cctype>
#include <cstdlib>
#include <cstring>
#include <string>

namespace cvk {
namespace {

struct Key {
  const char* name;
  int Tuning::*field;
};

#define CVK_KEY(f) {#f, &Tuning::f}
const Key kKeys[] = {
    CVK_KEY(trace), CVK_KEY(host_threads), CVK_KEY(t64_nonpos), CVK_KEY(generic_rows),
    CVK_KEY(max_chunks), CVK_KEY(emis_overlap), CVK_KEY(host_sums), CVK_KEY(no_trace), CVK_KEY(no_resume),
    CVK_KEY(no_side), CVK_KEY(chain_par), CVK_KEY(chain_old), CVK_KEY(chain_par_force),
    CVK_KEY(chain_spec), CVK_KEY(chain_spec_kernel), CVK_KEY(chain_copy_overlap), CVK_KEY(chain_cert_fused),
    CVK_KEY(chain_parts), CVK_KEY(chain_tail), CVK_KEY(chain_tail_div), CVK_KEY(chain_spec_prio), CVK_KEY(chain_pin_obs), CVK_KEY(chain_pin_path), CVK_KEY(t64_s),
    CVK_KEY(t64_512), CVK_KEY(t64_1024), CVK_KEY(t64_wg), CVK_KEY(t64_wg_force),
    CVK_KEY(t64_rs), CVK_KEY(t64_w2), CVK_KEY(t64_wave), CVK_KEY(t64_bal),
    CVK_KEY(t64_cp_s), CVK_KEY(t64_cp_w), CVK_KEY(t64_cp_pf), CVK_KEY(t64_bt_pf),
    CVK_KEY(t64_lo_every), CVK_KEY(t64_fixed_first), CVK_KEY(t64_fixed_chunks), CVK_KEY(t64_few),
    CVK_KEY(generic_s), CVK_KEY(generic_split), CVK_KEY(generic_split_k), CVK_KEY(generic_wide),
    CVK_KEY(generic_wide_min), CVK_KEY(generic_prio), CVK_KEY(wide_s), CVK_KEY(ext_wide_min),
    CVK_KEY(chain_wide), CVK_KEY(chain_wide_min), CVK_KEY(f32_onebar), CVK_KEY(bw_global),
    CVK_KEY(bw_perseq), CVK_KEY(bw_gemm_path), CVK_KEY(bw_chunk_elems), CVK_KEY(bw_max_waves),
};
#undef CVK_KEY

const Key* find(const char* key) {
  if (!key) return nullptr;
  for (const Key& k : kKeys)
    if (std::strcmp(k.name, key) == 0) return &k;
  return nullptr;
}

const Tuning kDefaults{};
thread_local const Tuning* t_cur = nullptr;
thread_local Tuning t_copy;
thread_local int t_depth = 0;

}

const Tuning& tuning() { return t_cur ? *t_cur : kDefaults; }

void tuning_enter(const Tuning& t) {
  if (t_depth++ == 0) {
    t_copy = t;
    t_cur = &t_copy;
  }
}

void tuning_leave() {
  if (t_depth > 0 && --t_depth == 0) t_cur = nullptr;
}

TuningOverride::TuningOverride(int Tuning::*field, int value) : field_(field), saved_(0), on_(t_cur != nullptr) {
  if (!on_) return;
  saved_ = t_copy.*field_;
  t_copy.*field_ = value;
}

TuningOverride::~TuningOverride() {
  if (on_ && t_cur) t_copy.*field_ = saved_;
}

Tuning tuning_from_env() {
  Tuning t;
  for (const Key& k : kKeys) {
    std::string var = "CV_";
    for (const char* p = k.name; *p; ++p) var += (char)std::toupper((unsigned char)*p);
    const char* e = std::getenv(var.c_str());
    if (!e || !*e) continue;
    char* end = nullptr;
    const long v = std::strtol(e, &end, 10);
    if (end != e) t.*(k.field) = (int)v;
  }
  return t;
}

bool tuning_set(Tuning& t, const char* key, int64_t value) {
  const Key* k = find(key);
  if (!k || value < INT32_MIN || value > INT32_MAX) return false;
  t.*(k->field) = (int)value;
  return true;
}

bool tuning_get(const Tuning& t, const char* key, int64_t* value) {
  const Key* k = find(key);
  if (!k || !value) return false;
  *value = t.*(k->field);
  return true;
}

const char* tuning_key(int i) {
  return i >= 0 && i < (int)(sizeof(kKeys) / sizeof(kKeys[0])) ? kKeys[i].name : nullptr;
}

}
```

consistent-viterbi_amd/csrc/tuning.h:

```cpp
#pragma once

#include <cstdint>

namespace cvk {

struct Tuning {
  int trace = 0;
  int host_threads = 0;
  int t64_nonpos = 1;
  int generic_rows = 1;
  int max_chunks = 8;
  int emis_overlap = 0;
  int host_sums = 0;
  int no_trace = 0;
  int no_resume = 0;
  int no_side = 0;
  int chain_par = 1;
  int chain_old = 0;
  int chain_par_force = 0;
  int chain_spec = 1;
  int chain_spec_kernel = 0;
  int chain_copy_overlap = 1;
  int chain_cert_fused = 1;
  int chain_parts = 1;
  int chain_tail = 2;
  int chain_tail_div = 2;
  int chain_spec_prio = 3;
  int chain_pin_obs = 0;
  int chain_pin_path = 0;
  int t64_s = 0;
  int t64_512 = -1;
  int t64_1024 = -1;
  int t64_wg = 1;
  int t64_wg_force = 0;
  int t64_rs = 1;
  int t64_w2 = 1;
  int t64_few = -1;
  int t64_wave = 1;
  int t64_bal = 8;
  int t64_cp_s = 0;
  int t64_cp_pf = 0;
  int t64_cp_w = 0;
  int t64_bt_pf = 0;
  int t64_lo_every = 8;
  int t64_fixed_first = 16777216;
  int t64_fixed_chunks = 8;
  int generic_s = 0;
  int generic_split = 0;
  int generic_split_k = 0;
  int generic_wide = 1;
  int generic_wide_min = 0;
  int generic_prio = 0;
  int wide_s = 0;
  int ext_wide_min = 0;
  int chain_wide = 1;
  int chain_wide_min = 0;
  int f32_onebar = 1;
  int bw_global = 0;
  int bw_perseq = 0;
  int bw_gemm_path = 0;
  int bw_chunk_elems = 0;
  int bw_max_waves = 0;
};

const Tuning& tuning();
void tuning_enter(const Tuning& t);
void tuning_leave();
struct TuningOverride {
  TuningOverride(int Tuning::*field, int value);
  ~TuningOverride();
  TuningOverride(const TuningOverride&) = delete;
  TuningOverride& operator=(const TuningOverride&) = delete;

 private:
  int Tuning::*field_;
  int saved_;
  bool on_;
};
struct TuningScope {
  explicit TuningScope(const Tuning& t) { tuning_enter(t); }
  ~TuningScope() { tuning_leave(); }
  TuningScope(const TuningScope&) = delete;
  TuningScope& operator=(const TuningScope&) = delete;
};

Tuning tuning_from_env();
bool tuning_set(Tuning& t, const char* key, int64_t value);
bool tuning_get(const Tuning& t, const char* key, int64_t* value);
const char* tuning_key(int i);

}
```

consistent-viterbi_amd/cviterbi/__init__.py:

```python
from ._lib import CVError, EXPORTS, LIB_PATH
from .hmm import HMM, tuning_keys
from .decode import (constrained_pairs, constrained_partials, constrained_select, decode, decode_batch, decode_batch_device, decode_constrained_device, decode_constrained_exchange,
                     decode_constrained, decode_forced_components, decode_superseq_cp, device_memory, last_suffix_traced, last_fixed_first_stats, last_superseq_stats, last_t64_stats, last_timing, timing_begin,
                     timing_end)
from .emissions import decode_emissions, decode_emissions_device
from .emissions import posterior_emissions, posterior_emissions_device, score_emissions
from .fit import fit_mle, fit_train, last_fit_stats
from .kbest import kbest_batch, kbest_batch_device
from .posterior import posterior_batch, posterior_batch_device, score_batch
from .sample import sample_batch, sample_batch_device, uniform
from .solver import (Constraints, GpuSolver, Solver, SuperSequence, load_sequences, load_tags,
                     write_output)
```

consistent-viterbi_amd/cviterbi/_lib.py:

```python
from __future__ import annotations

import ctypes
import os

_HERE = os.path.dirname(os.path.abspath(__file__))
LIB_PATH = os.environ.get("CV_LIB_PATH") or os.path.join(_HERE, "libcviterbi.so")

(CV_OK, CV_EINVAL, CV_EDEVICE, CV_ENOMEM, CV_EINFEASIBLE, CV_EIO, CV_EPARSE, CV_EUNSUPPORTED, CV_EINTERNAL,
 CV_ELIMIT) = range(10)
STATUS_NAMES = {0: "CV_OK", 1: "CV_EINVAL", 2: "CV_EDEVICE", 3: "CV_ENOMEM", 4: "CV_EINFEASIBLE", 5: "CV_EIO",
                6: "CV_EPARSE", 7: "CV_EUNSUPPORTED", 8: "CV_EINTERNAL", 9: "CV_ELIMIT"}
SEQ_OK, SEQ_INFEASIBLE, SEQ_EMPTY, SEQ_BADOBS = 0, 1, 2, 3
DTYPE_F32, DTYPE_F64 = 0, 1
ASSOC_VITERBI, ASSOC_CP, ASSOC_DP, ASSOC_DECODE = 0, 1, 2, 3
KERNEL_AUTO, KERNEL_TRELLIS, KERNEL_GENERIC, KERNEL_TRELLIS_F64 = 0, 1, 2, 3
FLAG_NO_PAIR = 0x4
FLAG_NO_WAVE = 0x8
FLAG_NO_T64 = 0x10
FLAG_SERIAL = 0x2


EXPORTS = [
    "cv_last_error", "cv_version", "cv_abi_version", "cv_device_count", "cv_device_memory", "cv_opts_init",
    "cv_hmm_create", "cv_hmm_from_json", "cv_hmm_write_json", "cv_hmm_destroy", "cv_hmm_nstates", "cv_hmm_nobs",
    "cv_hmm_ndims", "cv_hmm_bdims", "cv_obs_flatten", "cv_hmm_init_prob", "cv_hmm_init_probs",
    "cv_hmm_transition_prob", "cv_hmm_transitions_to", "cv_hmm_emit_prob", "cv_hmm_emit_probs",
    "cv_decode_batch", "cv_decode_batch_device", "cv_last_timing", "cv_timing_begin", "cv_timing_end",
    "cv_decode_constrained", "cv_decode_constrained_device", "cv_last_suffix_traced", "cv_decode_constrained_exchange",
    "cv_constrained_pairs", "cv_constrained_partials", "cv_constrained_select", "cv_decode_forced_components", "cv_viterbi_decode",
    "cv_decode_superseq_cp", "cv_last_superseq_stats",
    "cv_solver_create", "cv_solver_solve", "cv_solver_get_solution", "cv_solver_get_objective",
    "cv_solver_get_name", "cv_solver_get_explored_nodes", "cv_solver_destroy",
    "cv_hmm_fit_mle", "cv_hmm_fit_train", "cv_solver_write_cfn",
    "cv_hmm_set_tuning", "cv_hmm_get_tuning", "cv_tuning_key", "cv_hmm_release_workspaces",
    "cv_posterior_batch", "cv_posterior_batch_device",
    "cv_kbest_batch", "cv_kbest_batch_device",
    "cv_decode_emissions", "cv_decode_emissions_device",
    "cv_posterior_emissions", "cv_posterior_emissions_device",
    "cv_sample_batch", "cv_sample_batch_device",
    "cv_last_t64_stats", "cv_last_fixed_first_stats", "cv_hmm_fit_last_stats",
]


class CVError(RuntimeError):
    def __init__(self, status, message):
        super().__init__(f"{STATUS_NAMES.get(status, status)}: {message}")
        self.status = status


class HmmDesc(ctypes.Structure):
    _fields_ = [("nstates", ctypes.c_int32), ("ndims", ctypes.c_int32), ("bdims", ctypes.c_void_p),
                ("pi", ctypes.c_void_p), ("a", ctypes.c_void_p), ("b", ctypes.c_void_p), ("device", ctypes.c_int32)]


class Opts(ctypes.Structure):
    _fields_ = [("dtype", ctypes.c_int32), ("assoc", ctypes.c_int32), ("kernel", ctypes.c_int32),
                ("rescore_f64", ctypes.c_int32), ("stream", ctypes.c_void_p), ("workspace_bytes", ctypes.c_uint64),
                ("flags", ctypes.c_uint32), ("forced", ctypes.c_void_p)]


class Timing(ctypes.Structure):
    _fields_ = [("fwd_ms", ctypes.c_double), ("bt_ms", ctypes.c_double), ("total_ms", ctypes.c_double),
                ("launches", ctypes.c_int64), ("kernel", ctypes.c_int32), ("padded_states", ctypes.c_int32),
                ("mfma_tiles", ctypes.c_int32)]


class SuperSeqDesc(ctypes.Structure):
    _fields_ = [("nseq", ctypes.c_int64), ("offsets", ctypes.c_void_p), ("obs", ctypes.c_void_p),
                ("seq_id", ctypes.c_void_p), ("component", ctypes.c_void_p), ("active", ctypes.c_void_p)]


_lib = None


def lib():
    global _lib
    if _lib is not None:
        return _lib
    if not os.path.exists(LIB_PATH):
        raise CVError(CV_EDEVICE, f"{LIB_PATH} not built (python -c 'import __graft_entry__ as g; g.build()')")
    try:
        import torch
    except ImportError:
        pass
    L = ctypes.CDLL(LIB_PATH)
    P, I32, I64, D, S = ctypes.c_void_p, ctypes.c_int32, ctypes.c_int64, ctypes.c_double, ctypes.c_int
    sig = {
        "cv_last_error": ([], ctypes.c_char_p),
        "cv_version": ([], ctypes.c_char_p),
        "cv_abi_version": ([], I32),
        "cv_device_count": ([], I32),
        "cv_opts_init": ([P], None),
        "cv_hmm_create": ([P, P], S),
        "cv_hmm_from_json": ([ctypes.c_char_p, I32, P], S),
        "cv_hmm_write_json": ([P, ctypes.c_char_p], S),
        "cv_hmm_destroy": ([P], None),
        "cv_hmm_set_tuning": ([P, ctypes.c_char_p, I64], S),
        "cv_hmm_get_tuning": ([P, ctypes.c_char_p, P], S),
        "cv_tuning_key": ([I32], ctypes.c_char_p),
        "cv_hmm_release_workspaces": ([P], S),
        "cv_hmm_nstates": ([P], I32),
        "cv_hmm_nobs": ([P], I64),
        "cv_hmm_ndims": ([P], I32),
        "cv_hmm_bdims": ([P, P], S),
        "cv_obs_flatten": ([P, P, P], S),
        "cv_hmm_init_prob": ([P, I32, I64], D),
        "cv_hmm_init_probs": ([P, I64, P], S),
        "cv_hmm_transition_prob": ([P, I32, I32, I64], D),
        "cv_hmm_transitions_to": ([P, I32, P], S),
        "cv_hmm_emit_prob": ([P, I32, I64], D),
        "cv_hmm_emit_probs": ([P, I64, P], S),
        "cv_decode_batch": ([P, I64, P, P, P, P, P, P], S),
        "cv_decode_batch_device": ([P, I64, P, P, P, P, P, P, P], S),
        "cv_posterior_batch": ([P, I64, P, P, P, P, P, P, P], S),
        "cv_posterior_batch_device": ([P, I64, P, P, P, P, P, P, P, P], S),
        "cv_sample_batch": ([P, I64, P, P, I32, ctypes.c_uint64, I64, P, P, P, P, P], S),
        "cv_sample_batch_device": ([P, I64, P, P, P, I32, ctypes.c_uint64, I64, P, P, P, P, P], S),
        "cv_kbest_batch": ([P, I64, P, P, I32, P, P, P, P, P], S),
        "cv_kbest_batch_device": ([P, I64, P, P, P, I32, P, P, P, P, P], S),
        "cv_decode_emissions": ([P, I64, P, P, I64, P, P, P, P], S),
        "cv_decode_emissions_device": ([P, I64, P, P, P, I64, P, P, P, P], S),
        "cv_posterior_emissions": ([P, I64, P, P, I64, P, P, P, P, P], S),
        "cv_posterior_emissions_device": ([P, I64, P, P, P, I64, P, P, P, P, P], S),
        "cv_last_timing": ([P, P], S),
        "cv_timing_begin": ([P], S),
        "cv_timing_end": ([P, P], S),
        "cv_last_suffix_traced": ([P, P], S),
        "cv_decode_constrained": ([P, I64, P, P, P, I32, P, P, P, P, P, P], S),
        "cv_decode_constrained_device": ([P, I64, P, P, P, P, I32, P, P, P, P, P, P], S),
        "cv_decode_constrained_exchange": ([P, I64, P, P, P, I32, I64, P, P, P, P, P, P, P, P, P, P], S),
        "cv_constrained_pairs": ([I64, P, P, I32, P, I64, P], S),
        "cv_constrained_partials": ([P, I64, P, P, P, I32, I64, P, P, P], S),
        "cv_constrained_select": ([I32, I32, I64, P, P, P, P], S),
        "cv_decode_forced_components": ([P, I64, P, P, P, I32, P, P, P, P, P, P], S),
        "cv_viterbi_decode": ([P, I64, P, P], S),
        "cv_decode_superseq_cp": ([P, I64, P, P, P, P], S),
        "cv_last_superseq_stats": ([P, P], S),
        "cv_last_t64_stats": ([P, P, I32], I32),
        "cv_last_fixed_first_stats": ([P, P, I32], I32),
        "cv_device_memory": ([P, P], S),
        "cv_solver_create": ([ctypes.c_char_p, P, P, P], S),
        "cv_solver_solve": ([P], S),
        "cv_solver_get_solution": ([P, P, P], S),
        "cv_solver_get_objective": ([P, P], S),
        "cv_solver_get_name": ([P], ctypes.c_char_p),
        "cv_solver_get_explored_nodes": ([P, P], S),
        "cv_solver_destroy": ([P], None),
        "cv_solver_write_cfn": ([P, ctypes.c_char_p, P], S),
        "cv_hmm_fit_mle": ([I32, I64, I64, P, P, P, I32, P, P, P], S),
        "cv_hmm_fit_train": ([I32, I64, I64, P, P, P, I32, D, I32, P, P, P, P], S),
        "cv_hmm_fit_last_stats": ([P, I32], I32),
    }
    for name, (args, res) in sig.items():
        f = getattr(L, name)
        f.argtypes = args
        f.restype = res
    _lib = L
    return L


def check(status):
    if status != CV_OK:
        raise CVError(status, lib().cv_last_error().decode())


def opts(dtype=DTYPE_F32, assoc=ASSOC_VITERBI, kernel=KERNEL_AUTO, rescore_f64=True, stream=None,
         workspace_bytes=0, flags=0):
    o = Opts()
    lib().cv_opts_init(ctypes.byref(o))
    o.dtype, o.assoc, o.kernel, o.rescore_f64 = dtype, assoc, kernel, int(bool(rescore_f64))
    o.stream = stream
    o.workspace_bytes = workspace_bytes
    o.flags = flags
    return o
```

consistent-viterbi_amd/cviterbi/decode.py:

```python
from __future__ import annotations

import ctypes

import numpy as np

from . import _lib as L
from .hmm import HMM

_DT = {"f32": L.DTYPE_F32, "f64": L.DTYPE_F64, np.float32: L.DTYPE_F32, np.float64: L.DTYPE_F64}
_ASSOC = {"viterbi": L.ASSOC_VITERBI, "cp": L.ASSOC_CP, "dp": L.ASSOC_DP, "decode": L.ASSOC_DECODE}
_KERNEL = {"auto": L.KERNEL_AUTO, "trellis": L.KERNEL_TRELLIS, "generic": L.KERNEL_GENERIC,
           "trellis_f64": L.KERNEL_TRELLIS_F64}


def _p(x):
    return x.ctypes.data_as(ctypes.c_void_p)


def make_opts(dtype="f64", assoc="viterbi", kernel="auto", rescore_f64=True, stream=None, workspace_bytes=0,
              variant=None, serial=False):
    flags = L.FLAG_SERIAL if serial else 0
    if variant == "valu1":
        flags |= L.FLAG_NO_PAIR | L.FLAG_NO_WAVE
    elif variant == "nowave":
# ... 65 lines not shown
        pairs = constrained_pairs(offsets, component, ncomp)
    pairs = np.ascontiguousarray(pairs, np.int32).reshape(-1, 2)
    part = np.zeros(max(partial_words(hmm.nstates(), ncomp, len(pairs)), 1), np.int64)
    o = make_opts(dtype, "viterbi", "auto", True)
    L.check(L.lib().cv_constrained_partials(hmm.handle, offsets.shape[0] - 1, _p(offsets), _p(obs), _p(component),
                                            int(ncomp), len(pairs), _p(pairs) if len(pairs) else None,
                                            ctypes.byref(o), _p(part)))
    return part[:partial_words(hmm.nstates(), ncomp, len(pairs))]


def constrained_select(nstates: int, ncomp: int, partials, pairs=None):
    partials = np.ascontiguousarray(partials, np.int64)
    pairs = np.zeros((0, 2), np.int32) if pairs is None else np.ascontiguousarray(pairs, np.int32).reshape(-1, 2)
    if partials.size != partial_words(nstates, ncomp, len(pairs)):
        raise ValueError("partials size does not match (nstates, ncomp, pairs)")
    states = np.full(max(ncomp, 1), -1, np.int32)
    ex = ctypes.c_uint64()
    L.check(L.lib().cv_constrained_select(int(nstates), int(ncomp), len(pairs), _p(pairs) if len(pairs) else None,
                                          _p(partials), _p(states), ctypes.byref(ex)))
    return states[:ncomp], ex.value


def decode_forced_components(hmm: HMM, offsets, obs, component, comp_state, rescore_f64=True, dtype="f64"):
    offsets = np.ascontiguousarray(offsets, np.int64)
    obs = np.ascontiguousarray(obs, np.int32)
    component = np.ascontiguousarray(component, np.int32)
    cs = np.ascontiguousarray(comp_state, np.int32)
    nseq = offsets.shape[0] - 1
    path = np.zeros(int(offsets[-1]), np.int32)
    score = np.zeros(nseq, np.float64)
    status = np.zeros(nseq, np.uint8)
    obj = ctypes.c_double()
    o = make_opts(dtype, "viterbi", "auto", rescore_f64)
    L.check(L.lib().cv_decode_forced_components(hmm.handle, nseq, _p(offsets), _p(obs), _p(component), len(cs),
                                                _p(cs) if len(cs) else None, ctypes.byref(o), _p(path), _p(score),
                                                _p(status), ctypes.byref(obj)))
    return path, score, status, obj.value


def decode_batch_device(hmm: HMM, offsets_dev, obs_dev, path_dev, score_dev, status_dev, offsets_host=None,
                        dtype="f64", assoc="viterbi", kernel="auto", rescore_f64=True, stream=None,
                        workspace_bytes=0, variant=None, serial=False):
    def ptr(x):
        if x is None:
            return None
        return x.data_ptr() if hasattr(x, "data_ptr") else int(x)

    nseq = (len(offsets_host) if offsets_host is not None else offsets_dev.numel()) - 1
    oh = None
    if offsets_host is not None:
        oh = np.ascontiguousarray(offsets_host, np.int64)
    o = make_opts(dtype, assoc, kernel, rescore_f64, stream, workspace_bytes, variant, serial)
    L.check(L.lib().cv_decode_batch_device(hmm.handle, nseq, _p(oh) if oh is not None else None, ptr(offsets_dev),
                                           ptr(obs_dev), ctypes.byref(o), ptr(path_dev), ptr(score_dev),
                                           ptr(status_dev)))


EXCHANGE_FN = ctypes.CFUNCTYPE(ctypes.c_int32, ctypes.POINTER(ctypes.c_int64), ctypes.c_int64, ctypes.c_void_p)


def decode_constrained_exchange(hmm: HMM, offsets, obs, component, ncomp, pairs, exchange=None, rescore_f64=True,
                                dtype="f64"):
    offsets = np.ascontiguousarray(offsets, np.int64)
    obs = np.ascontiguousarray(obs, np.int32)
    component = np.ascontiguousarray(component, np.int32)
    pairs = np.ascontiguousarray(pairs, np.int32).reshape(-1, 2)
    nseq = offsets.shape[0] - 1
    path = np.zeros(max(int(offsets[-1]), 1), np.int32)
    score = np.zeros(max(nseq, 1), np.float64)
    status = np.zeros(max(nseq, 1), np.uint8)
    states = np.full(max(ncomp, 1), -1, np.int32)
    explored, obj = ctypes.c_uint64(), ctypes.c_double()
    err = []

    def cb(words, n, _ctx):
        try:
            w = np.ctypeslib.as_array(words, shape=(n,))
            w[:] = np.asarray(exchange(w.copy()), np.int64).reshape(-1)
            return 0
        except Exception as e:
            err.append(e)
            return 1

    fn = EXCHANGE_FN(cb) if exchange is not None else None
    o = make_opts(dtype, "viterbi", "auto", rescore_f64)
    st = L.lib().cv_decode_constrained_exchange(hmm.handle, nseq, _p(offsets), _p(obs), _p(component), int(ncomp),
                                                len(pairs), _p(pairs) if len(pairs) else None,
                                                ctypes.cast(fn, ctypes.c_void_p) if fn else None, None,
                                                ctypes.byref(o), _p(path), _p(score), _p(status), _p(states),
                                                ctypes.byref(explored), ctypes.byref(obj))
    if err:
        raise err[0]
    L.check(st)
    return (path[:int(offsets[-1])], score[:nseq], status[:nseq], states[:ncomp], explored.value, obj.value)


def decode_constrained_device(hmm: HMM, offsets_host, offsets_dev, obs_dev, component, path_dev, score_dev, status_dev,
                              ncomp=None, rescore_f64=True, stream=None, workspace_bytes=0, dtype="f64"):
    def ptr(x):
        return x.data_ptr() if hasattr(x, "data_ptr") else int(x)

    oh = np.ascontiguousarray(offsets_host, np.int64)
    component = np.ascontiguousarray(component, np.int32)
    if ncomp is None:
        ncomp = int(component.max()) + 1 if component.size else 0
    states = np.full(max(ncomp, 1), -1, np.int32)
    obj = ctypes.c_double()
    o = make_opts(dtype, "viterbi", "auto", rescore_f64, stream, workspace_bytes)
    L.check(L.lib().cv_decode_constrained_device(hmm.handle, oh.shape[0] - 1, _p(oh), ptr(offsets_dev), ptr(obs_dev),
                                                 _p(component), int(ncomp), ctypes.byref(o), ptr(path_dev),
                                                 ptr(score_dev), ptr(status_dev), _p(states), ctypes.byref(obj)))
    return states[:ncomp], obj.value


def decode_superseq_cp(hmm: HMM, offsets, obs):
    offsets = np.ascontiguousarray(offsets, np.int64)
    obs = np.ascontiguousarray(obs, np.int32)
    path = np.zeros(max(int(offsets[-1] - offsets[0]), 1), np.int32)
    obj = ctypes.c_double()
    L.check(L.lib().cv_decode_superseq_cp(hmm.handle, offsets.shape[0] - 1, _p(offsets), _p(obs), _p(path),
                                          ctypes.byref(obj)))
    return path[:int(offsets[-1] - offsets[0])], obj.value


def last_superseq_stats(hmm: HMM) -> dict:
    out = (ctypes.c_int64 * 9)()
    L.check(L.lib().cv_last_superseq_stats(hmm.handle, out))
    return dict(parallel=bool(out[0]), certified=out[1], rerun=out[2], runs=out[3], quantised=out[4],
                speculated=out[5], spec_batches=out[6], gathered=out[7], path_waits=out[8])


T64_STATS = ("lo_every", "events", "scans", "levels", "overflows", "mismatches", "max_need", "sequences")


def last_t64_stats(hmm: HMM) -> dict:
    out = (ctypes.c_int64 * len(T64_STATS))()
    n = L.lib().cv_last_t64_stats(hmm.handle, out, len(T64_STATS))
    if n < 0:
        L.check(L.CV_EINVAL)
    return {k: int(out[i]) for i, k in enumerate(T64_STATS[:n])}


FIXED_FIRST_STATS = ("engaged", "certified", "fallback", "pinned")


def last_fixed_first_stats(hmm: HMM) -> dict:
    out = (ctypes.c_int64 * len(FIXED_FIRST_STATS))()
    n = L.lib().cv_last_fixed_first_stats(hmm.handle, out, len(FIXED_FIRST_STATS))
    if n < 0:
        L.check(L.CV_EINVAL)
    return {k: int(out[i]) for i, k in enumerate(FIXED_FIRST_STATS[:n])}


def device_memory() -> dict:
    cur, peak = ctypes.c_int64(), ctypes.c_int64()
    L.check(L.lib().cv_device_memory(ctypes.byref(cur), ctypes.byref(peak)))
    return dict(current=cur.value, peak=peak.value)


def _timing_dict(t):
    return dict(fwd_ms=t.fwd_ms, bt_ms=t.bt_ms, total_ms=t.total_ms, launches=t.launches,
                kernel={1: "trellis", 2: "generic", 3: "trellis_f64"}.get(t.kernel, "none"), padded_states=t.padded_states,
                seqs_per_wave=t.mfma_tiles)


def last_suffix_traced(hmm: HMM) -> int:
    n = ctypes.c_int64()
    L.check(L.lib().cv_last_suffix_traced(hmm.handle, ctypes.byref(n)))
    return n.value


def last_timing(hmm: HMM) -> dict:
    t = L.Timing()
    L.check(L.lib().cv_last_timing(hmm.handle, ctypes.byref(t)))
    return _timing_dict(t)


def timing_begin(hmm: HMM):
    L.check(L.lib().cv_timing_begin(hmm.handle))


def timing_end(hmm: HMM) -> dict:
    t = L.Timing()
    L.check(L.lib().cv_timing_end(hmm.handle, ctypes.byref(t)))
    return _timing_dict(t)


def decode(sequence, hmm: HMM):
    obs = np.ascontiguousarray([hmm.flat(o) for o in sequence], np.int32)
    path = np.zeros(obs.shape[0], np.int32)
    L.check(L.lib().cv_viterbi_decode(hmm.handle, obs.shape[0], _p(obs), _p(path)))
    return path
```

include/cviterbi.h:

```cpp
#ifndef CVITERBI_H
#define CVITERBI_H

#include <stddef.h>
#include <stdint.h>

#ifdef __cplusplus
extern "C" {
#endif

#define CV_API __attribute__((visibility("default")))
#define CV_ABI_VERSION 1

typedef enum cv_status {
  CV_OK = 0,
  CV_EINVAL = 1,
  CV_EDEVICE = 2,
  CV_ENOMEM = 3,
  CV_EINFEASIBLE = 4,
  CV_EIO = 5,
  CV_EPARSE = 6,
  CV_EUNSUPPORTED = 7,
  CV_EINTERNAL = 8,
  CV_ELIMIT = 9
} cv_status;

enum { CV_SEQ_OK = 0, CV_SEQ_INFEASIBLE = 1, CV_SEQ_EMPTY = 2, CV_SEQ_BADOBS = 3 };

enum { CV_DTYPE_F32 = 0, CV_DTYPE_F64 = 1 };

enum { CV_ASSOC_VITERBI = 0, CV_ASSOC_CP = 1, CV_ASSOC_DP = 2, CV_ASSOC_DECODE = 3 };

enum { CV_KERNEL_AUTO = 0, CV_KERNEL_TRELLIS = 1, CV_KERNEL_GENERIC = 2, CV_KERNEL_TRELLIS_F64 = 3 };

#define CV_FLAG_SERIAL 0x2u
#define CV_FLAG_NO_PAIR 0x4u
#define CV_FLAG_NO_WAVE 0x8u
#define CV_FLAG_NO_T64 0x10u

typedef struct cv_hmm cv_hmm;
typedef struct cv_solver cv_solver;

typedef struct cv_hmm_desc {
  int32_t nstates;
  int32_t ndims;
  const int64_t* bdims;
  const double* pi;
  const double* a;
  const double* b;
  int32_t device;
} cv_hmm_desc;

typedef struct cv_opts {
  int32_t dtype;
  int32_t assoc;
  int32_t kernel;
  int32_t rescore_f64;
  void* stream;
  uint64_t workspace_bytes;
  uint32_t flags;
  const int32_t* forced;
} cv_opts;

typedef struct cv_timing {
  double fwd_ms;
  double bt_ms;
  double total_ms;
  int64_t launches;
  int32_t kernel;
  int32_t padded_states;
  int32_t mfma_tiles;
} cv_timing;

typedef struct cv_superseq_desc {
  int64_t nseq;
  const int64_t* offsets;
  const int32_t* obs;
  const int64_t* seq_id;
  const int32_t* component;
  const uint8_t* active;
} cv_superseq_desc;

CV_API const char* cv_last_error(void);
CV_API const char* cv_version(void);
CV_API int32_t cv_abi_version(void);
CV_API int32_t cv_device_count(void);
CV_API cv_status cv_device_memory(int64_t* current_bytes, int64_t* peak_bytes);
CV_API void cv_opts_init(cv_opts* opts);

CV_API cv_status cv_hmm_create(const cv_hmm_desc* desc, cv_hmm** out);
CV_API cv_status cv_hmm_from_json(const char* path, int32_t device, cv_hmm** out);
CV_API cv_status cv_hmm_write_json(const cv_hmm* h, const char* path);
CV_API void cv_hmm_destroy(cv_hmm* h);
CV_API cv_status cv_hmm_release_workspaces(cv_hmm* h);
CV_API cv_status cv_hmm_set_tuning(cv_hmm* h, const char* key, int64_t value);
CV_API cv_status cv_hmm_get_tuning(const cv_hmm* h, const char* key, int64_t* value);
CV_API const char* cv_tuning_key(int32_t i);

CV_API int32_t cv_hmm_nstates(const cv_hmm* h);
CV_API int64_t cv_hmm_nobs(const cv_hmm* h);
CV_API int32_t cv_hmm_ndims(const cv_hmm* h);
CV_API cv_status cv_hmm_bdims(const cv_hmm* h, int64_t* bdims_out );
CV_API cv_status cv_obs_flatten(const cv_hmm* h, const int64_t* value , int64_t* flat_out);
CV_API double cv_hmm_init_prob(const cv_hmm* h, int32_t state, int64_t obs);
CV_API cv_status cv_hmm_init_probs(const cv_hmm* h, int64_t obs, double* out);
CV_API double cv_hmm_transition_prob(const cv_hmm* h, int32_t from, int32_t to, int64_t obs);
CV_API cv_status cv_hmm_transitions_to(const cv_hmm* h, int32_t to, double* out);
CV_API double cv_hmm_emit_prob(const cv_hmm* h, int32_t state, int64_t obs);
CV_API cv_status cv_hmm_emit_probs(const cv_hmm* h, int64_t obs, double* out);

CV_API cv_status cv_decode_batch(cv_hmm* h, int64_t nseq, const int64_t* offsets, const int32_t* obs,
                                 const cv_opts* opts, int32_t* path_out, double* score_out,
                                 uint8_t* status_out);
CV_API cv_status cv_decode_batch_device(cv_hmm* h, int64_t nseq, const int64_t* offsets_host,
                                        const int64_t* offsets_dev, const int32_t* obs_dev,
                                        const cv_opts* opts, int32_t* path_dev, double* score_dev,
                                        uint8_t* status_dev);
CV_API int32_t cv_last_t64_stats(const cv_hmm* h, int64_t* out, int32_t n);
CV_API int32_t cv_last_fixed_first_stats(const cv_hmm* h, int64_t* out, int32_t n);
CV_API cv_status cv_last_timing(cv_hmm* h, cv_timing* out);
CV_API cv_status cv_timing_begin(cv_hmm* h);
CV_API cv_status cv_timing_end(cv_hmm* h, cv_timing* out);
CV_API cv_status cv_decode_constrained(cv_hmm* h, int64_t nseq, const int64_t* offsets, const int32_t* obs,
                                       const int32_t* component, int32_t ncomp, const cv_opts* opts,
                                       int32_t* path_out, double* score_out, uint8_t* status_out,
                                       int32_t* comp_state_out, double* objective_out);
CV_API cv_status cv_decode_constrained_device(cv_hmm* h, int64_t nseq, const int64_t* offsets_host,
                                              const int64_t* offsets_dev, const int32_t* obs_dev,
                                              const int32_t* component, int32_t ncomp, const cv_opts* opts,
                                              int32_t* path_dev, double* score_dev, uint8_t* status_dev,
                                              int32_t* comp_state_out, double* objective_out);
CV_API cv_status cv_last_suffix_traced(const cv_hmm* h, int64_t* out);
#define CV_PARTIAL_WORDS(nstates, ncomp, npairs) \
  ((int64_t)(ncomp) * (5 * (int64_t)(nstates) + 1) + (int64_t)(npairs) * (5 * (int64_t)(nstates) * (nstates) + 1))
CV_API cv_status cv_constrained_pairs(int64_t nseq, const int64_t* offsets, const int32_t* component, int32_t ncomp,
                                      int32_t* pairs_out, int64_t cap_pairs, int64_t* npairs_out);
CV_API cv_status cv_constrained_partials(cv_hmm* h, int64_t nseq, const int64_t* offsets, const int32_t* obs,
                                         const int32_t* component, int32_t ncomp, int64_t npairs,
                                         const int32_t* pairs, const cv_opts* opts, int64_t* partials_out);
CV_API cv_status cv_constrained_select(int32_t nstates, int32_t ncomp, int64_t npairs, const int32_t* pairs,
                                       const int64_t* partials, int32_t* comp_state_out, uint64_t* explored_out);
CV_API cv_status cv_decode_forced_components(cv_hmm* h, int64_t nseq, const int64_t* offsets, const int32_t* obs,
                                             const int32_t* component, int32_t ncomp, const int32_t* comp_state,
                                             const cv_opts* opts, int32_t* path_out, double* score_out,
                                             uint8_t* status_out, double* objective_out);
typedef int32_t (*cv_exchange_fn)(int64_t* words, int64_t nwords, void* ctx);
CV_API cv_status cv_decode_constrained_exchange(cv_hmm* h, int64_t nseq, const int64_t* offsets, const int32_t* obs,
                                                const int32_t* component, int32_t ncomp, int64_t npairs,
                                                const int32_t* pairs, cv_exchange_fn exchange, void* ctx,
                                                const cv_opts* opts, int32_t* path_out, double* score_out,
                                                uint8_t* status_out, int32_t* comp_state_out,
                                                uint64_t* explored_out, double* objective_out);
CV_API cv_status cv_viterbi_decode(cv_hmm* h, int64_t T, const int32_t* obs, int32_t* path_out);
CV_API cv_status cv_decode_superseq_cp(cv_hmm* h, int64_t nseq, const int64_t* offsets, const int32_t* obs,
                                       int32_t* path_out, double* objective_out);
CV_API cv_status cv_last_superseq_stats(const cv_hmm* h, int64_t* out);

CV_API cv_status cv_posterior_batch(cv_hmm* h, int64_t nseq, const int64_t* offsets, const int32_t* obs,
                                    const cv_opts* opts, double* loglik_out, int32_t* path_out,
                                    double* gamma_out, uint8_t* status_out);
CV_API cv_status cv_posterior_batch_device(cv_hmm* h, int64_t nseq, const int64_t* offsets_host,
                                           const int64_t* offsets_dev, const int32_t* obs_dev, const cv_opts* opts,
                                           double* loglik_dev, int32_t* path_dev, double* gamma_dev,
                                           uint8_t* status_dev);

CV_API cv_status cv_sample_batch(cv_hmm* h, int64_t nseq, const int64_t* offsets, const int32_t* obs,
                                 int32_t draws, uint64_t seed, int64_t seq_base, const cv_opts* opts,
                                 int32_t* path_out , double* score_out ,
                                 double* loglik_out , uint8_t* status_out );
CV_API cv_status cv_sample_batch_device(cv_hmm* h, int64_t nseq, const int64_t* offsets_host,
                                        const int64_t* offsets_dev, const int32_t* obs_dev, int32_t draws,
                                        uint64_t seed, int64_t seq_base, const cv_opts* opts, int32_t* path_dev,
                                        double* score_dev, double* loglik_dev, uint8_t* status_dev);

CV_API cv_status cv_kbest_batch(cv_hmm* h, int64_t nseq, const int64_t* offsets, const int32_t* obs,
                                int32_t k, const cv_opts* opts, int32_t* path_out ,
                                double* score_out , int32_t* count_out ,
                                uint8_t* status_out );
CV_API cv_status cv_kbest_batch_device(cv_hmm* h, int64_t nseq, const int64_t* offsets_host,
                                       const int64_t* offsets_dev, const int32_t* obs_dev, int32_t k,
                                       const cv_opts* opts, int32_t* path_dev, double* score_dev,
                                       int32_t* count_dev, uint8_t* status_dev);

CV_API cv_status cv_decode_emissions(cv_hmm* h, int64_t nseq, const int64_t* offsets, const double* emis,
                                     int64_t ld, const cv_opts* opts, int32_t* path_out, double* score_out,
                                     uint8_t* status_out);
CV_API cv_status cv_decode_emissions_device(cv_hmm* h, int64_t nseq, const int64_t* offsets_host,
                                            const int64_t* offsets_dev, const double* emis_dev, int64_t ld,
                                            const cv_opts* opts, int32_t* path_dev, double* score_dev,
                                            uint8_t* status_dev);

CV_API cv_status cv_posterior_emissions(cv_hmm* h, int64_t nseq, const int64_t* offsets, const double* emis,
                                        int64_t ld, const cv_opts* opts, double* loglik_out, int32_t* path_out,
                                        double* gamma_out, uint8_t* status_out);
CV_API cv_status cv_posterior_emissions_device(cv_hmm* h, int64_t nseq, const int64_t* offsets_host,
                                               const int64_t* offsets_dev, const double* emis_dev, int64_t ld,
                                               const cv_opts* opts, double* loglik_dev, int32_t* path_dev,
                                               double* gamma_dev, uint8_t* status_dev);

CV_API cv_status cv_solver_create(const char* kind, cv_hmm* h, const cv_superseq_desc* seq, cv_solver** out);
CV_API cv_status cv_solver_solve(cv_solver* s);
CV_API cv_status cv_solver_get_solution(const cv_solver* s, const int32_t** sol, int64_t* len);
CV_API cv_status cv_solver_get_objective(const cv_solver* s, double* obj);
CV_API const char* cv_solver_get_name(const cv_solver* s);
CV_API cv_status cv_solver_get_explored_nodes(const cv_solver* s, uint64_t* n);
CV_API void cv_solver_destroy(cv_solver* s);
CV_API cv_status cv_solver_write_cfn(cv_solver* s, const char* path, uint64_t* compile_ms);

CV_API cv_status cv_hmm_fit_mle(int32_t nstates, int64_t nobs, int64_t nseq, const int64_t* offsets,
                                const int32_t* obs, const int32_t* tags, int32_t device, double* pi, double* a,
                                double* b);
CV_API cv_status cv_hmm_fit_train(int32_t nstates, int64_t nobs, int64_t nseq, const int64_t* offsets,
                                  const int32_t* obs, const int32_t* tags, int32_t max_iter, double tol,
                                  int32_t device, double* pi, double* a, double* b, int32_t* iters_out);
CV_API int32_t cv_hmm_fit_last_stats(int64_t* out, int32_t n);

#ifdef __cplusplus
}
#endif
#endif
```

Before: 75.36 billion.

## Add rounded-up f32 first pass with certified f64 rescoring for Viterbi decode

Adds a new first-pass decoder that runs the trellis forward in float32. Scores are shifted by per-state and per-observation offsets and rounded upward, so each f32 value is an upper bound on the true score. A backtrack kernel records per-step residuals, and an f64 scoring kernel checks a margin bound to certify each path, falling back to the exact path when certification fails. This pass is preferred over the existing fixed-point first pass when enabled, which it is by default for large batches. It aims for cheaper f32 arithmetic than integer fixed-point, at the cost of extra mu/r buffers and possibly more sequences that fail certification and need the fallback.

```diff
diff --git a/consistent-viterbi_amd/csrc/cviterbi.cpp b/consistent-viterbi_amd/csrc/cviterbi.cpp
--- a/consistent-viterbi_amd/csrc/cviterbi.cpp
+++ b/consistent-viterbi_amd/csrc/cviterbi.cpp
@@ -236,6 +236,11 @@
   std::vector<int64_t> fx_idx_host;
   bool fx_pinned = false;
   int64_t fx_last[4] = {0, 0, 0, 0};
+  int ru_state = -1;
+  DevBuf ru_aimg, ru_pi, ru_et, ru_at, ru_ca, ru_cb;
+  double ru_ks = 0.0;
+  DevBuf ru_mu, ru_r, ru_e;
+  int fx_last_kind = 0;
   DevBuf q_pi0;
   bool g32_ready = false;
   DevBuf d_pi32, d_a32, d_et32;
@@ -1671,6 +1676,7 @@
     h->nonpos_cache = -1;
     h->t64_ready = false;
     h->fx_state = -1;
+    h->ru_state = -1;
   }
   return CV_OK;
 }
@@ -1695,7 +1701,8 @@
                     &h->chainb.sobs, &h->chainb.spath, &h->chainb.sres, &h->chainb.sinit, &h->chainb.slast,
                     &h->chainb.spsi, &h->ps_rows,
                     &h->ps_order, &h->ps_kshift, &h->st_gamma, &h->kb_bp, &h->kb_last, &h->kb_order, &h->kb_end, &h->st_count,
-                    &h->st_emis, &h->fx_cert, &h->fx_idx, &h->fx_obs2, &h->fx_path2, &h->fx_score2, &h->fx_status2})
+                    &h->st_emis, &h->fx_cert, &h->fx_idx, &h->fx_obs2, &h->fx_path2, &h->fx_score2, &h->fx_status2,
+                    &h->ru_mu, &h->ru_r, &h->ru_e})
     b->release();
   h->fx_cert_pin.release();
   h->sm_pin.release();
@@ -1821,23 +1828,118 @@
   return CV_OK;
 }
 
+static float ru_sum32(double x, double y) {
+  const double s = x + y;
+  if (!std::isfinite(s)) return (float)s;
+  const double bb = s - x;
+  const double e = (x - (s - bb)) + (y - bb);
+  float f = (float)s;
+  if ((double)f < s || ((double)f == s && e > 0.0)) f = std::nextafter(f, std::numeric_limits<float>::infinity());
+  return f;
+}
+static double ru_grid(double x) {
+  return std::isfinite(x) ? std::nearbyint(x * 65536.0) / 65536.0 : 0.0;
+}
+
+static cv_status ensure_ru_tables(cv_hmm* h) {
+  if (h->ru_state >= 0) return CV_OK;
+  const int np = cvk::trellis_padded_states(h->N);
+  if (!cvk::fix_supported(np) || !model_nonpos(h)) {
+    h->ru_state = 0;
+    return CV_OK;
+  }
+  const int N = h->N;
+  const int64_t V = h->V;
+  const int R = np / 8;
+  const float ninf = -std::numeric_limits<float>::infinity();
+  std::vector<double> ca((size_t)N), cb((size_t)V);
+  for (int j = 0; j < N; ++j) {
+    double m = -INFINITY;
+    for (int i = 0; i < N; ++i) m = std::max(m, h->a[(size_t)i * N + j]);
+    ca[(size_t)j] = ru_grid(m);
+  }
+  for (int64_t o = 0; o < V; ++o) {
+    double m = -INFINITY;
+    for (int j = 0; j < N; ++j) m = std::max(m, h->b[(size_t)j * V + o] + ca[(size_t)j]);
+    cb[(size_t)o] = ru_grid(m);
+  }
+  double smax = 0.0;
+  for (double x : ca) smax = std::max(smax, std::fabs(x));
+  for (double x : cb) smax = std::max(smax, std::fabs(x));
+  if (!(smax < 1073741824.0)) {
+    h->ru_state = 0;
+    return CV_OK;
+  }
+  auto A = [&](int i, int j) -> float {
+    return (i < N && j < N) ? ru_sum32(h->a[(size_t)i * N + j], -ca[(size_t)j]) : ninf;
+  };
+  std::vector<float> img((size_t)np * np), pi((size_t)np, ninf), at((size_t)np * np, ninf), et((size_t)V * np, ninf);
+  for (int w = 0; w < np / 16; ++w)
+    for (int q = 0; q < R / 2; ++q)
+      for (int lane = 0; lane < 64; ++lane) {
+        const int rg = lane & 7, cp = lane >> 3, j0 = 16 * w + 2 * cp, r0 = rg * R + 2 * q;
+        float* dst = &img[(((size_t)w * (R / 2) + q) * 64 + lane) * 4];
+        dst[0] = A(r0, j0);
+        dst[1] = A(r0, j0 + 1);
+        dst[2] = A(r0 + 1, j0);
+        dst[3] = A(r0 + 1, j0 + 1);
+      }
+  for (int j = 0; j < N; ++j) pi[(size_t)j] = ru_sum32(h->pi[(size_t)j], -ca[(size_t)j]);
+  for (int i = 0; i < N; ++i)
+    for (int j = 0; j < N; ++j) at[(size_t)j * np + i] = A(i, j);
+  parallel_ranges(N, [&](int, int64_t lo, int64_t hi) {
+    for (int64_t j = lo; j < hi; ++j)
+      for (int64_t o = 0; o < V; ++o)
+        et[(size_t)o * np + j] = ru_sum32(h->b[(size_t)j * V + o], ca[(size_t)j] - cb[(size_t)o]);
+  }, std::max<int64_t>(1, 4096 / std::max<int64_t>(V, 1)));
+  double wmax = 0.0;
+  for (const std::vector<double>* v : {&h->pi, &h->a, &h->b}) {
+    double m = 0.0;
+    for (double x : *v)
+      if (std::isfinite(x)) m = std::max(m, std::fabs(x));
+    wmax += m;
+  }
+  h->ru_ks = 4.0 * std::ldexp(1.0, -53) * wmax;
+  cv_status st;
+  if ((st = upload(h->ru_aimg, img.data(), img.size() * 4)) != CV_OK) return st;
+  if ((st = upload(h->ru_pi, pi.data(), pi.size() * 4)) != CV_OK) return st;
+  if ((st = upload(h->ru_at, at.data(), at.size() * 4)) != CV_OK) return st;
+  if ((st = upload(h->ru_et, et.data(), et.size() * 4)) != CV_OK) return st;
+  if ((st = upload(h->ru_ca, ca.data(), ca.size() * 8)) != CV_OK) return st;
+  if ((st = upload(h->ru_cb, cb.data(), cb.size() * 8)) != CV_OK) return st;
+  h->ru_state = 1;
+  return CV_OK;
+}
+
 static cv_status fixed_first_decode(cv_hmm* h, int64_t nseq, const int64_t* offsets_host, const int64_t* offsets_dev,
                                     const int32_t* obs_dev, const cv_opts& o, int32_t* path_dev, double* score_dev,
                                     uint8_t* status_dev, hipStream_t stream, bool* done) {
   *done = false;
   h->fx_last[0] = h->fx_last[1] = h->fx_last[2] = 0;
   h->fx_last[3] = h->fx_pinned ? 1 : 0;
-  const int64_t min_elems = h->tuning.t64_fixed_first;
-  if (min_elems <= 0 || h->fx_pinned || h->fx_state == 0 || nseq < 2 || nseq > INT32_MAX) return CV_OK;
+  h->fx_last_kind = 0;
+  enum FirstPass { kNone = 0, kFix = 1, kRu = 2 };
+  const int64_t min_fix = h->tuning.t64_fixed_first, min_ru = h->tuning.t64_f32ru_first;
+  const bool fix_open = min_fix > 0 && h->fx_state != 0, ru_open = min_ru > 0 && h->ru_state != 0;
+  if ((!fix_open && !ru_open) || h->fx_pinned || nseq < 2 || nseq > INT32_MAX) return CV_OK;
   if (o.dtype != CV_DTYPE_F64 || o.assoc != CV_ASSOC_VITERBI || o.forced || o.flags != 0 ||
       (o.kernel != CV_KERNEL_AUTO && o.kernel != CV_KERNEL_TRELLIS_F64))
     return CV_OK;
   std::vector<int64_t> off_copy;
   cv_status st = host_offsets(nseq, offsets_host, offsets_dev, off_copy, stream);
   if (st != CV_OK) return st;
-  if (offsets_host[nseq] - offsets_host[0] < min_elems) return CV_OK;
-  if ((st = ensure_fix_tables(h)) != CV_OK) return st;
-  if (h->fx_state != 1) return CV_OK;
+  const int64_t elems = offsets_host[nseq] - offsets_host[0];
+  FirstPass pass = kNone;
+  if (ru_open && elems >= min_ru) {
+    if ((st = ensure_ru_tables(h)) != CV_OK) return st;
+    if (h->ru_state == 1) pass = kRu;
+  }
+  if (pass == kNone && fix_open && elems >= min_fix) {
+    if ((st = ensure_fix_tables(h)) != CV_OK) return st;
+    if (h->fx_state == 1) pass = kFix;
+  }
+  if (pass == kNone) return CV_OK;
+  const bool ru = pass == kRu;
   if ((st = ensure_f64_tables(h)) != CV_OK) return st;
   const int np = cvk::trellis_padded_states(h->N);
 
@@ -1866,6 +1968,12 @@
     cvplan::longest_first(offsets_host, chunks, h->order_host.data(), npair.data(), h->sort_pos);
     if ((st = upload_order(h->ws_order, h->order_pin, h->order_host.data(), nseq, stream, &order_dev)) != CV_OK) return st;
   }
+  if (ru) {
+    const size_t ne = (size_t)std::max<int64_t>(offsets_host[nseq], 1);
+    if ((st = h->ru_mu.ensure(ne * 4)) != CV_OK) return st;
+    if ((st = h->ru_r.ensure(ne * 4)) != CV_OK) return st;
+    if ((st = h->ru_e.ensure((size_t)nseq * 4)) != CV_OK) return st;
+  }
   HIP_TRY(hipMemsetAsync(h->fx_cert.p, 0, (size_t)nseq, stream));
 
   const bool acc_was = h->acc_on;
@@ -1897,20 +2005,41 @@
     hipEvent_t f0 = e4[0], f1 = e4[1], b0 = e4[2], b1 = e4[3];
     if (!serial && ci >= 2) HIP_TRY(hipStreamWaitEvent(stream, h->ev[eb + 4 * (ci - 2) + 3], 0));
     HIP_TRY(hipEventRecord(f0, stream));
-    cvk::FixFwdArgs fa{};
-    fa.a_img = h->fx_aimg.as<int32_t>();
-    fa.pi = h->fx_pi.as<int32_t>();
-    fa.et = h->fx_et.as<int32_t>();
-    fa.offsets = offsets_dev;
-    fa.obs = obs_dev;
-    fa.order = order_dev;
-    fa.seq_begin = c.first;
-    fa.rows = reinterpret_cast<int32_t*>(h->ws_main.as<unsigned char>() + (nbuf == 2 ? ci % 2 : 0) * buf_bytes);
-    fa.row_elem_base = offsets_host[c.first];
-    fa.cert = h->fx_cert.as<uint8_t>();
-    fa.nobs = (int)h->V;
-    hipError_t err = cvk::launch_fix_fwd2(np, fa, np2, stream);
-    if (err != hipSuccess) return set_err(CV_EDEVICE, "fixed-point forward launch failed: %s", hipGetErrorString(err));
+    void* const rows = h->ws_main.as<unsigned char>() + (nbuf == 2 ? ci % 2 : 0) * buf_bytes;
+    const int64_t row_base = offsets_host[c.first];
+    uint8_t* const cert_dev = h->fx_cert.as<uint8_t>();
+    hipError_t err;
+    if (ru) {
+      cvk::RuFwdArgs fa{};
+      fa.a_img = h->ru_aimg.as<float>();
+      fa.pi = h->ru_pi.as<float>();
+      fa.et = h->ru_et.as<float>();
+      fa.offsets = offsets_dev;
+      fa.obs = obs_dev;
+      fa.order = order_dev;
+      fa.seq_begin = c.first;
+      fa.rows = static_cast<float*>(rows);
+      fa.row_elem_base = row_base;
+      fa.mu = h->ru_mu.as<float>();
+      fa.cert = cert_dev;
+      fa.nobs = (int)h->V;
+      err = cvk::launch_ru_fwd2(np, fa, np2, stream);
+    } else {
+      cvk::FixFwdArgs fa{};
+      fa.a_img = h->fx_aimg.as<int32_t>();
+      fa.pi = h->fx_pi.as<int32_t>();
+      fa.et = h->fx_et.as<int32_t>();
+      fa.offsets = offsets_dev;
+      fa.obs = obs_dev;
+      fa.order = order_dev;
+      fa.seq_begin = c.first;
+      fa.rows = static_cast<int32_t*>(rows);
+      fa.row_elem_base = row_base;
+      fa.cert = cert_dev;
+      fa.nobs = (int)h->V;
+      err = cvk::launch_fix_fwd2(np, fa, np2, stream);
+    }
+    if (err != hipSuccess) return set_err(CV_EDEVICE, "first-pass forward launch failed: %s", hipGetErrorString(err));
     HIP_TRY(hipEventRecord(f1, stream));
     if (!serial) {
       HIP_TRY(hipStreamWaitEvent(bts, f1, 0));
@@ -1918,33 +2047,71 @@
     }
     HIP_TRY(hipEventRecord(b0, bts));
     const int reserve = (serial || ci + 1 == chunks.size()) ? 0 : 100 * 1024;
-    cvk::FixBtArgs ba{};
-    ba.rows = fa.rows;
-    ba.row_elem_base = fa.row_elem_base;
-    ba.at = h->fx_at.as<int32_t>();
-    ba.offsets = offsets_dev;
-    ba.order = order_dev;
-    ba.seq_begin = c.first;
-    ba.seq_end = c.first + 2 * np2;
-    ba.gain = h->fx_gain;
-    ba.path = path_dev;
-    ba.cert = fa.cert;
-    err = cvk::launch_fix_bt(np, ba, bts, reserve);
-    if (err == hipSuccess) {
-      cvk::FixScoreArgs ra{};
-      ra.path = path_dev;
-      ra.obs = obs_dev;
-      ra.offsets = offsets_dev;
-      ra.seq_begin = c.first;
-      ra.seq_end = c.second;
-      ra.nstates = h->N;
-      ra.pi64 = h->d_pi64.as<double>();
-      ra.a64 = h->d_a64.as<double>();
-      ra.et64 = h->d_et64.as<double>();
-      ra.cert = fa.cert;
-      ra.score = score_dev;
-      ra.status = status_dev;
-      err = cvk::launch_fix_score(ra, bts, reserve);
+    if (ru) {
+      cvk::RuBtArgs ba{};
+      ba.rows = static_cast<const float*>(rows);
+      ba.row_elem_base = row_base;
+      ba.at = h->ru_at.as<float>();
+      ba.offsets = offsets_dev;
+      ba.order = order_dev;
+      ba.seq_begin = c.first;
+      ba.seq_end = c.first + 2 * np2;
+      ba.path = path_dev;
+      ba.r = h->ru_r.as<float>();
+      ba.e_last = h->ru_e.as<float>();
+      ba.cert = cert_dev;
+      err = cvk::launch_ru_bt(np, ba, bts, reserve);
+      if (err == hipSuccess) {
+        cvk::RuScoreArgs ra{};
+        ra.path = path_dev;
+        ra.obs = obs_dev;
+        ra.offsets = offsets_dev;
+        ra.seq_begin = c.first;
+        ra.seq_end = c.second;
+        ra.nstates = h->N;
+        ra.pi64 = h->d_pi64.as<double>();
+        ra.a64 = h->d_a64.as<double>();
+        ra.et64 = h->d_et64.as<double>();
+        ra.ca = h->ru_ca.as<double>();
+        ra.cb = h->ru_cb.as<double>();
+        ra.mu = h->ru_mu.as<float>();
+        ra.r = h->ru_r.as<float>();
+        ra.e_last = h->ru_e.as<float>();
+        ra.ks = h->ru_ks;
+        ra.cert = cert_dev;
+        ra.score = score_dev;
+        ra.status = status_dev;
+        err = cvk::launch_ru_score(ra, bts, reserve);
+      }
+    } else {
+      cvk::FixBtArgs ba{};
+      ba.rows = static_cast<const int32_t*>(rows);
+      ba.row_elem_base = row_base;
+      ba.at = h->fx_at.as<int32_t>();
+      ba.offsets = offsets_dev;
+      ba.order = order_dev;
+      ba.seq_begin = c.first;
+      ba.seq_end = c.first + 2 * np2;
+      ba.gain = h->fx_gain;
+      ba.path = path_dev;
+      ba.cert = cert_dev;
+      err = cvk::launch_fix_bt(np, ba, bts, reserve);
+      if (err == hipSuccess) {
+        cvk::FixScoreArgs ra{};
+        ra.path = path_dev;
+        ra.obs = obs_dev;
+        ra.offsets = offsets_dev;
+        ra.seq_begin = c.first;
+        ra.seq_end = c.second;
+        ra.nstates = h->N;
+        ra.pi64 = h->d_pi64.as<double>();
+        ra.a64 = h->d_a64.as<double>();
+        ra.et64 = h->d_et64.as<double>();
+        ra.cert = cert_dev;
+        ra.score = score_dev;
+        ra.status = status_dev;
+        err = cvk::launch_fix_score(ra, bts, reserve);
+      }
     }
     if (err != hipSuccess) return set_err(CV_EDEVICE, "fixed-point backtrack launch failed: %s", hipGetErrorString(err));
     HIP_TRY(hipEventRecord(b1, bts));
@@ -1962,6 +2129,7 @@
   int64_t nfb = 0, nfail = 0;
   for (int64_t s = 0; s < nseq; ++s) nfb += cert[s] != 1, nfail += cert[s] == 2;
   h->fx_last[0] = 1;
+  h->fx_last_kind = (int)pass;
   h->fx_last[1] = nseq - nfb;
   h->fx_last[2] = nfb;
   h->fx_last[3] = 0;
@@ -3599,6 +3767,78 @@
   }
   for (int32_t q = 0; q < n && q < 4; ++q) out[q] = h->fx_last[q];
   return 4;
+}
+
+CV_API int32_t cv_last_first_pass_kind(const cv_hmm* h) {
+  if (!h) {
+    set_err(CV_EINVAL, "null handle");
+    return -1;
+  }
+  return h->fx_last_kind;
+}
+
+CV_API cv_status cv_f32ru_trace(cv_hmm* h, int64_t nseq, int64_t T, const int32_t* obs, float* rows, float* mu,
+                                float* r, float* e_last, int32_t* path) {
+  if (!h || !obs || !rows || !mu || !r || !e_last || !path) return set_err(CV_EINVAL, "null argument");
+  if (nseq < 2 || T < 1 || nseq * T > (1 << 22)) return set_err(CV_EINVAL, "bad batch shape");
+  CV_LOCK(h);
+  cv_status st = set_device(h);
+  if (st != CV_OK) return st;
+  for (int64_t e = 0; e < nseq * T; ++e)
+    if (obs[e] < 0 || obs[e] >= h->V) return set_err(CV_EINVAL, "observation out of range");
+  if ((st = ensure_ru_tables(h)) != CV_OK) return st;
+  if (h->ru_state != 1) return set_err(CV_EINVAL, "the model is outside the round-up pass's range");
+  const int np = cvk::trellis_padded_states(h->N);
+  const size_t ne = (size_t)(nseq * T);
+  std::vector<int64_t> off((size_t)nseq + 1);
+  for (int64_t s = 0; s <= nseq; ++s) off[(size_t)s] = s * T;
+  DevBuf d_off, d_obs, d_rows, d_mu, d_r, d_e, d_path, d_cert;
+  if ((st = upload(d_off, off.data(), off.size() * 8)) != CV_OK) return st;
+  if ((st = upload(d_obs, obs, ne * 4)) != CV_OK) return st;
+  if ((st = d_rows.ensure(ne * np * 4)) != CV_OK) return st;
+  if ((st = d_mu.ensure(ne * 4)) != CV_OK) return st;
+  if ((st = d_r.ensure(ne * 4)) != CV_OK) return st;
+  if ((st = d_e.ensure((size_t)nseq * 4)) != CV_OK) return st;
+  if ((st = d_path.ensure(ne * 4)) != CV_OK) return st;
+  if ((st = d_cert.ensure((size_t)nseq)) != CV_OK) return st;
+  hipStream_t stream = h->stream;
+  HIP_TRY(hipMemsetAsync(d_cert.p, 0, (size_t)nseq, stream));
+  HIP_TRY(hipMemsetAsync(d_mu.p, 0, ne * 4, stream));
+  HIP_TRY(hipMemsetAsync(d_r.p, 0, ne * 4, stream));
+  HIP_TRY(hipMemsetAsync(d_rows.p, 0, ne * np * 4, stream));
+  HIP_TRY(hipMemsetAsync(d_path.p, 0, ne * 4, stream));
+  HIP_TRY(hipMemsetAsync(d_e.p, 0, (size_t)nseq * 4, stream));
+  cvk::RuFwdArgs fa{};
+  fa.a_img = h->ru_aimg.as<float>();
+  fa.pi = h->ru_pi.as<float>();
+  fa.et = h->ru_et.as<float>();
+  fa.offsets = d_off.as<int64_t>();
+  fa.obs = d_obs.as<int32_t>();
+  fa.rows = d_rows.as<float>();
+  fa.mu = d_mu.as<float>();
+  fa.cert = d_cert.as<uint8_t>();
+  fa.nobs = (int)h->V;
+  hipError_t err = cvk::launch_ru_fwd2(np, fa, nseq / 2, stream);
+  cvk::RuBtArgs ba{};
+  ba.rows = fa.rows;
+  ba.at = h->ru_at.as<float>();
+  ba.offsets = fa.offsets;
+  ba.seq_end = nseq - (nseq & 1);
+  ba.path = d_path.as<int32_t>();
+  ba.r = d_r.as<float>();
+  ba.e_last = d_e.as<float>();
+  ba.cert = fa.cert;
+  if (err == hipSuccess) err = cvk::launch_ru_bt(np, ba, stream, 0);
+  if (err != hipSuccess) return set_err(CV_EDEVICE, "round-up pass launch failed: %s", hipGetErrorString(err));
+  HIP_TRY(hipStreamSynchronize(stream));
+  std::vector<float> padded(ne * (size_t)np);
+  HIP_TRY(hipMemcpy(padded.data(), d_rows.p, padded.size() * 4, hipMemcpyDeviceToHost));
+  for (size_t e = 0; e < ne; ++e) std::memcpy(rows + e * (size_t)h->N, &padded[e * (size_t)np], (size_t)h->N * 4);
+  HIP_TRY(hipMemcpy(mu, d_mu.p, ne * 4, hipMemcpyDeviceToHost));
+  HIP_TRY(hipMemcpy(r, d_r.p, ne * 4, hipMemcpyDeviceToHost));
+  HIP_TRY(hipMemcpy(e_last, d_e.p, (size_t)nseq * 4, hipMemcpyDeviceToHost));
+  HIP_TRY(hipMemcpy(path, d_path.p, ne * 4, hipMemcpyDeviceToHost));
+  return CV_OK;
 }
 
 CV_API cv_status cv_last_suffix_traced(const cv_hmm* h, int64_t* out) {
diff --git a/consistent-viterbi_amd/csrc/kernels/trellis.h b/consistent-viterbi_amd/csrc/kernels/trellis.h
--- a/consistent-viterbi_amd/csrc/kernels/trellis.h
+++ b/consistent-viterbi_amd/csrc/kernels/trellis.h
@@ -106,6 +106,55 @@
 hipError_t launch_fix_fwd2(int np, const FixFwdArgs& fa, int64_t npairs, hipStream_t stream);
 hipError_t launch_fix_bt(int np, const FixBtArgs& ba, hipStream_t stream, int lds_reserve = 0);
 hipError_t launch_fix_score(const FixScoreArgs& r, hipStream_t stream, int lds_reserve = 0);
+
+struct RuFwdArgs {
+  const float* a_img;
+  const float* pi;
+  const float* et;
+  const int64_t* offsets;
+  const int32_t* obs;
+  const int32_t* order;
+  int64_t seq_begin;
+  float* rows;
+  int64_t row_elem_base;
+  float* mu;
+  uint8_t* cert;
+  int nobs;
+};
+struct RuBtArgs {
+  const float* rows;
+  int64_t row_elem_base;
+  const float* at;
+  const int64_t* offsets;
+  const int32_t* order;
+  int64_t seq_begin, seq_end;
+  int32_t* path;
+  float* r;
+  float* e_last;
+  uint8_t* cert;
+};
+struct RuScoreArgs {
+  const int32_t* path;
+  const int32_t* obs;
+  const int64_t* offsets;
+  int64_t seq_begin, seq_end;
+  int nstates;
+  const double* pi64;
+  const double* a64;
+  const double* et64;
+  const double* ca;
+  const double* cb;
+  const float* mu;
+  const float* r;
+  const float* e_last;
+  double ks;
+  uint8_t* cert;
+  double* score;
+  uint8_t* status;
+};
+hipError_t launch_ru_fwd2(int np, const RuFwdArgs& fa, int64_t npairs, hipStream_t stream);
+hipError_t launch_ru_bt(int np, const RuBtArgs& ba, hipStream_t stream, int lds_reserve = 0);
+hipError_t launch_ru_score(const RuScoreArgs& r, hipStream_t stream, int lds_reserve = 0);
 
 template <typename REAL>
 struct GenericFwdArgs {
diff --git a/consistent-viterbi_amd/csrc/kernels/trellis.hip b/consistent-viterbi_amd/csrc/kernels/trellis.hip
--- a/consistent-viterbi_amd/csrc/kernels/trellis.hip
+++ b/consistent-viterbi_amd/csrc/kernels/trellis.hip
@@ -1072,6 +1072,314 @@
     (void)hipFuncSetAttribute(reinterpret_cast<const void*>(&fix_score_f64), hipFuncAttributeMaxDynamicSharedMemorySize,
                               160 * 1024);
   hipLaunchKernelGGL(fix_score_f64, dim3((unsigned)((n + 63) / 64)), dim3(64), (size_t)lds_reserve, stream, r);
+  return hipGetLastError();
+}
+
+__device__ __forceinline__ void round_f32_up() {
+  __builtin_amdgcn_s_setreg(1 | (1 << 11), 1);
+  asm volatile("" ::: "memory");
+}
+__device__ __forceinline__ float dpp_max_half_mirror(float x) {
+  asm volatile("s_nop 1\n\tv_max_f32_dpp %0, %0, %0 row_half_mirror row_mask:0xf bank_mask:0xf" : "+v"(x));
+  return x;
+}
+
+template <int NP>
+__global__ __launch_bounds__(NP * 4) void trellis_fwd2_f32ru(RuFwdArgs args) {
+  using G = TrellisGeom<NP>;
+  constexpr int R = G::R;
+  constexpr int S = G::S;
+  static_assert(R % 8 == 0, "pair kernel needs NP % 64 == 0");
+  __shared__ __attribute__((aligned(16))) float lds[2][2][G::LDS_FLOATS];
+  __shared__ float mu[2][3];
+  round_f32_up();
+
+  const int lane = threadIdx.x & 63;
+  const int w = threadIdx.x >> 6;
+  const int rg = lane & 7;
+  const int cp = lane >> 3;
+  const int j0 = 16 * w + 2 * cp;
+  const bool hi = rg >= 4;
+  const unsigned jw = (unsigned)(j0 + (hi ? 1 : 0));
+
+  const int64_t slot = args.seq_begin + 2 * (int64_t)blockIdx.x;
+  const int64_t seqX = args.order ? (int64_t)args.order[slot] : slot;
+  const int64_t seqY = args.order ? (int64_t)args.order[slot + 1] : slot + 1;
+  const int64_t eX = args.offsets[seqX], eY = args.offsets[seqY];
+  const int T = (int)(args.offsets[seqX + 1] - eX);
+  if (T <= 0) return;
+  typedef const __attribute__((address_space(4))) int32_t* cobs_t;
+  const cobs_t obsX = (cobs_t)(args.obs + eX);
+  const cobs_t obsY = (cobs_t)(args.obs + eY);
+  float* const dX = args.rows + (eX - args.row_elem_base) * NP;
+  float* const dY = args.rows + (eY - args.row_elem_base) * NP;
+  float* const muX = args.mu + eX;
+  float* const muY = args.mu + eY;
+  const unsigned V = (unsigned)args.nobs;
+
+  if (threadIdx.x < 6) (&mu[0][0])[threadIdx.x] = ninf_f();
+  __builtin_amdgcn_s_setprio(3);
+  float a_reg[2 * R];
+  {
+    const float4* img = reinterpret_cast<const float4*>(args.a_img) + (size_t)w * (R / 2) * 64 + lane;
+#pragma unroll
+    for (int q = 0; q < R / 2; ++q) {
+      const float4 v = img[q * 64];
+      a_reg[4 * q + 0] = v.x;
+      a_reg[4 * q + 1] = v.y;
+      a_reg[4 * q + 2] = v.z;
+      a_reg[4 * q + 3] = v.w;
+    }
+  }
+  __builtin_amdgcn_s_waitcnt(0x0F70);
+  unsigned bad = 0;
+  auto obs_x = [&](int t) -> unsigned {
+    const unsigned o = (unsigned)obsX[t];
+    bad |= (o >= V) ? 1u : 0u;
+    return o < V ? o : 0u;
+  };
+  auto obs_y = [&](int t) -> unsigned {
+    const unsigned o = (unsigned)obsY[t];
+    bad |= (o >= V) ? 2u : 0u;
+    return o < V ? o : 0u;
+  };
+  auto et_row = [&](unsigned o) -> float { return (args.et + (size_t)o * NP)[jw]; };
+  const int lds_w = (j0 / R) * S + (j0 % R) + (hi ? 1 : 0);
+  auto clampT = [&](int t) { return t < T ? t : T - 1; };
+  typedef __attribute__((address_space(3))) float* lds_float_t;
+  auto post_max = [&](float v, float* dst) {
+    const float m = dpp_max_half_mirror(v);
+    if (rg == 0) asm volatile("ds_max_f32 %0, %1" : : "v"((unsigned)(size_t)(lds_float_t)dst), "v"(m) : "memory");
+  };
+  lds_barrier();
+
+  float eXr;
+  {
+    const float ex = et_row(obs_x(0)), ey = et_row(obs_y(0));
+    const float p = args.pi[jw];
+    eXr = et_row(obs_x(clampT(1)));
+    const float dx = p + ex, dy = p + ey;
+    lds[0][0][lds_w] = dx;
+    lds[1][0][lds_w] = dy;
+    dX[jw] = dx;
+    dY[jw] = dy;
+    post_max(dx, &mu[0][0]);
+    post_max(dy, &mu[1][0]);
+  }
+  float eYr;
+  unsigned oY = obs_y(clampT(1));
+  unsigned oX = obs_x(clampT(2));
+  lds_barrier();
+  constexpr int KB = R / 8;
+  auto ld8 = [&](const float* src, float4 (&dst)[2]) {
+    dst[0] = *reinterpret_cast<const float4*>(src);
+    dst[1] = *reinterpret_cast<const float4*>(src + 4);
+  };
+  float4 P[2], Q[2];
+  ld8(&lds[0][0][rg * S], P);
+
+  auto half = [&](const float* dsrc, const float* nsrc, float* ldst, float* drow, float* mus, float* mrow, int t,
+                  const float& e_use, float& e_load, unsigned& o_load, bool first, int t_obs) {
+    e_load = et_row(o_load);
+    const float mu_use = fmaxf(mus[(t + 2) % 3], -__FLT_MAX__);
+    if (threadIdx.x == 0) mus[(t + 1) % 3] = ninf_f();
+    if (KB > 1) ld8(dsrc + 8, Q);
+    float m0a = ninf_f(), m0b = ninf_f(), m1a = ninf_f(), m1b = ninf_f();
+    auto rows4 = [&](const float4& dd, int k, bool init) {
+      const float s00 = dd.x + a_reg[2 * k + 0], s01 = dd.x + a_reg[2 * k + 1];
+      const float s10 = dd.y + a_reg[2 * k + 2], s11 = dd.y + a_reg[2 * k + 3];
+      const float s20 = dd.z + a_reg[2 * k + 4], s21 = dd.z + a_reg[2 * k + 5];
+      const float s30 = dd.w + a_reg[2 * k + 6], s31 = dd.w + a_reg[2 * k + 7];
+      if (init) {
+        m0a = fmaxf(s00, s10);
+        m1a = fmaxf(s01, s11);
+        m0b = fmaxf(s20, s30);
+        m1b = fmaxf(s21, s31);
+      } else {
+        m0a = fmaxf(fmaxf(m0a, s00), s10);
+        m1a = fmaxf(fmaxf(m1a, s01), s11);
+        m0b = fmaxf(fmaxf(m0b, s20), s30);
+        m1b = fmaxf(fmaxf(m1b, s21), s31);
+      }
+    };
+#pragma unroll
+    for (int k = 0; k < KB; ++k) {
+      float4(&B)[2] = (k & 1) ? Q : P;
+      rows4(B[0], 8 * k, k == 0);
+      rows4(B[1], 8 * k + 4, false);
+      __builtin_amdgcn_sched_barrier(0);
+      if (k + 2 < KB)
+        ld8(dsrc + 8 * (k + 2), B);
+      else if (!(k & 1) && (k + 2 == KB || k + 1 == KB) && !first)
+        ld8(nsrc, P);
+      __builtin_amdgcn_sched_barrier(0);
+    }
+    const float m0 = fmaxf(m0a, m0b);
+    const float m1 = fmaxf(m1a, m1b);
+    float m = dpp_max_mirror(hi ? m1 : m0, hi ? m0 : m1);
+    m = dpp_max_xor1(m);
+    m = dpp_max_xor2(m);
+    const float dn = (m + e_use) - mu_use;
+    __builtin_amdgcn_sched_barrier(0);
+    o_load = first ? obs_y(t_obs) : obs_x(t_obs);
+    ldst[lds_w] = dn;
+    (drow + (size_t)t * NP)[jw] = dn;
+    mrow[t] = mu_use;
+    post_max(dn, &mus[t % 3]);
+    if (first) {
+      lds_barrier();
+      ld8(nsrc, P);
+    }
+  };
+  auto step = [&](int t) {
+    const int cur = (t - 1) & 1, nxt = t & 1;
+    half(&lds[0][cur][rg * S], &lds[1][cur][rg * S], &lds[0][nxt][0], dX, mu[0], muX, t, eXr, eYr, oY, true,
+         clampT(t + 1));
+    half(&lds[1][cur][rg * S], &lds[0][nxt][rg * S], &lds[1][nxt][0], dY, mu[1], muY, t, eYr, eXr, oX, false,
+         clampT(t + 2));
+  };
+  for (int t = 1; t < T; ++t) step(t);
+  if (bad && lane == 0 && w == 0) {
+    if (bad & 1u) args.cert[seqX] = CVK_SEQ_BADOBS;
+    if (bad & 2u) args.cert[seqY] = CVK_SEQ_BADOBS;
+  }
+}
+
+template <int NP>
+__global__ __launch_bounds__(256) void backtrack_f32ru(RuBtArgs args) {
+  constexpr int VL = NP / 64;
+  constexpr int PF = 8;
+  static_assert(VL == 4, "float4 rows");
+  round_f32_up();
+  const int lane = threadIdx.x & 63;
+  const int64_t slot = args.seq_begin + (int64_t)blockIdx.x * 4 + (threadIdx.x >> 6);
+  if (slot >= args.seq_end) return;
+  const int64_t seq = args.order ? (int64_t)args.order[slot] : slot;
+  const int64_t e0 = args.offsets[seq];
+  const int T = (int)(args.offsets[seq + 1] - e0);
+  if (T <= 0 || args.cert[seq] != 0) return;
+  int32_t* __restrict__ path = args.path + e0;
+  float* __restrict__ rout = args.r + e0;
+  const float* __restrict__ drow = args.rows + (e0 - args.row_elem_base) * NP + VL * lane;
+  const float* __restrict__ at = args.at + VL * lane;
+  auto load_row = [&](int r, float (&dst)[VL]) {
+    if (r >= 0) {
+      ld_vl<VL>(drow + (size_t)r * NP, dst);
+    } else {
+      dst[0] = dst[1] = dst[2] = dst[3] = ninf_f();
+    }
+  };
+  auto top2 = [&](const float (&s)[VL], float& M2) -> int {
+    const float M = wave_max(fmaxf(fmaxf(s[0], s[1]), fmaxf(s[2], s[3])));
+    const int win = first_argmax_vl<VL>(s, M, lane) & (NP - 1);
+    float o = ninf_f();
+#pragma unroll
+    for (int k = 0; k < VL; ++k) o = fmaxf(o, (VL * lane + k == win) ? ninf_f() : s[k]);
+    M2 = wave_max(o);
+    return win;
+  };
+  int cur;
+  float M2;
+  {
+    float last[VL];
+    load_row(T - 1, last);
+    cur = top2(last, M2);
+    if (lane == 0) args.e_last[seq] = M2;
+  }
+  int pathreg = 0;
+  float rreg = 0.0f;
+  if (lane == ((T - 1) & 63)) pathreg = cur;
+  if (((T - 1) & 63) == 0 && lane == 0) path[T - 1] = cur;
+  float ring[PF][VL];
+#pragma unroll
+  for (int u = 0; u < PF; ++u) load_row(T - 2 - u, ring[u]);
+  for (int base = T - 1; base >= 1; base -= PF) {
+#pragma unroll
+    for (int u = 0; u < PF; ++u) {
+      const int t = base - u;
+      if (t >= 1) {
+        float acol[VL];
+        ld_vl<VL>(at + (size_t)cur * NP, acol);
+        const float sv[VL] = {ring[u][0] + acol[0], ring[u][1] + acol[1], ring[u][2] + acol[2], ring[u][3] + acol[3]};
+        cur = top2(sv, M2);
+        if (lane == (t & 63)) rreg = M2;
+        if ((t & 63) == 0 && t + lane < T) rout[t + lane] = rreg;
+        const int tp = t - 1;
+        if (lane == (tp & 63)) pathreg = cur;
+        if ((tp & 63) == 0 && tp + lane < T) path[tp + lane] = pathreg;
+      }
+    }
+#pragma unroll
+    for (int u = 0; u < PF; ++u) load_row(base - PF - 1 - u, ring[u]);
+  }
+  if (lane >= 1 && lane < T && lane < 64) rout[lane] = rreg;
+  if (lane == 0) args.cert[seq] = 1;
+}
+
+__global__ __launch_bounds__(64) void ru_score_f64(RuScoreArgs r) {
+  const int64_t seq = r.seq_begin + (int64_t)blockIdx.x * 64 + threadIdx.x;
+  if (seq >= r.seq_end || r.cert[seq] != 1) return;
+  const int64_t e0 = r.offsets[seq];
+  const int T = (int)(r.offsets[seq + 1] - e0);
+  const int32_t* __restrict__ path = r.path + e0;
+  const int32_t* __restrict__ obs = r.obs + e0;
+  const float* __restrict__ mu = r.mu + e0;
+  const float* __restrict__ rr = r.r + e0;
+  const int N = r.nstates;
+  auto absfin = [](double x) { return __builtin_isinf(x) ? 0.0 : __builtin_fabs(x); };
+  auto sigma = [&](int n, double s) { return r.ks * (((double)n + 2.0) * ((double)n + 2.0)) + 0x1p-49 * s; };
+  int pp = path[0];
+  double L = r.pi64[pp] + r.et64[(size_t)obs[0] * N + pp];
+  double C = r.cb[obs[0]];
+  bool ok = true;
+  for (int t = 1; t < T; ++t) {
+    const int p = path[t];
+    const int o = obs[t];
+    const double rt = (double)rr[t], cap = r.ca[p];
+    const double lhs = L + r.a64[(size_t)pp * N + p];
+    const double rhs = (rt + cap) + C;
+    ok = ok && (lhs - rhs > sigma(t, absfin(rt) + __builtin_fabs(cap) + __builtin_fabs(C) + __builtin_fabs(lhs)));
+    L = lhs + r.et64[(size_t)o * N + p];
+    const double ct = r.cb[o], mt = (double)mu[t];
+    const double s = __builtin_fabs(C) + __builtin_fabs(ct) + __builtin_fabs(mt);
+    C = ((C + ct) + mt) + 0x1p-50 * s;
+    pp = p;
+  }
+  const double E = (double)r.e_last[seq];
+  ok = ok && (L - (E + C) > sigma(T, absfin(E) + __builtin_fabs(C) + __builtin_fabs(L)));
+  if (ok) {
+    r.score[seq] = L;
+    r.status[seq] = CVK_SEQ_OK;
+  } else {
+    r.cert[seq] = 2;
+  }
+}
+
+hipError_t launch_ru_fwd2(int np, const RuFwdArgs& fa, int64_t npairs, hipStream_t stream) {
+  if (npairs <= 0) return hipSuccess;
+  if (np != 256) return hipErrorInvalidValue;
+  hipLaunchKernelGGL((trellis_fwd2_f32ru<256>), dim3((unsigned)npairs), dim3(1024), 0, stream, fa);
+  return hipGetLastError();
+}
+
+hipError_t launch_ru_bt(int np, const RuBtArgs& ba, hipStream_t stream, int lds_reserve) {
+  const int64_t n = ba.seq_end - ba.seq_begin;
+  if (n <= 0) return hipSuccess;
+  if (np != 256) return hipErrorInvalidValue;
+  if (lds_reserve > 0)
+    (void)hipFuncSetAttribute(reinterpret_cast<const void*>(&backtrack_f32ru<256>),
+                              hipFuncAttributeMaxDynamicSharedMemorySize, 160 * 1024);
+  hipLaunchKernelGGL((backtrack_f32ru<256>), dim3((unsigned)((n + 3) / 4)), dim3(256), (size_t)lds_reserve, stream, ba);
+  return hipGetLastError();
+}
+
+hipError_t launch_ru_score(const RuScoreArgs& r, hipStream_t stream, int lds_reserve) {
+  const int64_t n = r.seq_end - r.seq_begin;
+  if (n <= 0) return hipSuccess;
+  if (lds_reserve > 0)
+    (void)hipFuncSetAttribute(reinterpret_cast<const void*>(&ru_score_f64), hipFuncAttributeMaxDynamicSharedMemorySize,
+                              160 * 1024);
+  hipLaunchKernelGGL(ru_score_f64, dim3((unsigned)((n + 63) / 64)), dim3(64), (size_t)lds_reserve, stream, r);
   return hipGetLastError();
 }
 
diff --git a/consistent-viterbi_amd/csrc/tuning.cpp b/consistent-viterbi_amd/csrc/tuning.cpp
--- a/consistent-viterbi_amd/csrc/tuning.cpp
+++ b/consistent-viterbi_amd/csrc/tuning.cpp
@@ -24,6 +24,7 @@
     CVK_KEY(t64_rs), CVK_KEY(t64_w2), CVK_KEY(t64_wave), CVK_KEY(t64_bal),
     CVK_KEY(t64_cp_s), CVK_KEY(t64_cp_w), CVK_KEY(t64_cp_pf), CVK_KEY(t64_bt_pf),
     CVK_KEY(t64_lo_every), CVK_KEY(t64_fixed_first), CVK_KEY(t64_fixed_chunks), CVK_KEY(t64_few),
+    CVK_KEY(t64_f32ru_first),
     CVK_KEY(generic_s), CVK_KEY(generic_split), CVK_KEY(generic_split_k), CVK_KEY(generic_wide),
     CVK_KEY(generic_wide_min), CVK_KEY(generic_prio), CVK_KEY(wide_s), CVK_KEY(ext_wide_min),
     CVK_KEY(chain_wide), CVK_KEY(chain_wide_min), CVK_KEY(f32_onebar), CVK_KEY(bw_global),
diff --git a/consistent-viterbi_amd/csrc/tuning.h b/consistent-viterbi_amd/csrc/tuning.h
--- a/consistent-viterbi_amd/csrc/tuning.h
+++ b/consistent-viterbi_amd/csrc/tuning.h
@@ -44,6 +44,7 @@
   int t64_bt_pf = 0;
   int t64_lo_every = 8;
   int t64_fixed_first = 16777216;
+  int t64_f32ru_first = 16777216;
   int t64_fixed_chunks = 8;
   int generic_s = 0;
   int generic_split = 0;
diff --git a/consistent-viterbi_amd/cviterbi/__init__.py b/consistent-viterbi_amd/cviterbi/__init__.py
--- a/consistent-viterbi_amd/cviterbi/__init__.py
+++ b/consistent-viterbi_amd/cviterbi/__init__.py
@@ -1,7 +1,7 @@
 from ._lib import CVError, EXPORTS, LIB_PATH
 from .hmm import HMM, tuning_keys
 from .decode import (constrained_pairs, constrained_partials, constrained_select, decode, decode_batch, decode_batch_device, decode_constrained_device, decode_constrained_exchange,
-                     decode_constrained, decode_forced_components, decode_superseq_cp, device_memory, last_suffix_traced, last_fixed_first_stats, last_superseq_stats, last_t64_stats, last_timing, timing_begin,
+                     decode_constrained, decode_forced_components, decode_superseq_cp, device_memory, f32ru_trace, last_first_pass_kind, last_suffix_traced, last_fixed_first_stats, last_superseq_stats, last_t64_stats, last_timing, timing_begin,
                      timing_end)
 from .emissions import decode_emissions, decode_emissions_device
 from .emissions import posterior_emissions, posterior_emissions_device, score_emissions
diff --git a/consistent-viterbi_amd/cviterbi/_lib.py b/consistent-viterbi_amd/cviterbi/_lib.py
--- a/consistent-viterbi_amd/cviterbi/_lib.py
+++ b/consistent-viterbi_amd/cviterbi/_lib.py
@@ -39,6 +39,7 @@
     "cv_posterior_emissions", "cv_posterior_emissions_device",
     "cv_sample_batch", "cv_sample_batch_device",
     "cv_last_t64_stats", "cv_last_fixed_first_stats", "cv_hmm_fit_last_stats",
+    "cv_last_first_pass_kind", "cv_f32ru_trace",
 ]
 
 
@@ -138,6 +139,8 @@
         "cv_last_superseq_stats": ([P, P], S),
         "cv_last_t64_stats": ([P, P, I32], I32),
         "cv_last_fixed_first_stats": ([P, P, I32], I32),
+        "cv_last_first_pass_kind": ([P], I32),
+        "cv_f32ru_trace": ([P, I64, I64, P, P, P, P, P, P], S),
         "cv_device_memory": ([P, P], S),
         "cv_solver_create": ([ctypes.c_char_p, P, P, P], S),
         "cv_solver_solve": ([P], S),
diff --git a/consistent-viterbi_amd/cviterbi/decode.py b/consistent-viterbi_amd/cviterbi/decode.py
--- a/consistent-viterbi_amd/cviterbi/decode.py
+++ b/consistent-viterbi_amd/cviterbi/decode.py
@@ -241,6 +241,28 @@
     return {k: int(out[i]) for i, k in enumerate(FIXED_FIRST_STATS[:n])}
 
 
+FIRST_PASS_KINDS = ("none", "fixed", "f32ru")
+
+
+def last_first_pass_kind(hmm: HMM) -> str:
+    k = L.lib().cv_last_first_pass_kind(hmm.handle)
+    if k < 0:
+        L.check(L.CV_EINVAL)
+    return FIRST_PASS_KINDS[k]
+
+
+def f32ru_trace(hmm: HMM, obs) -> dict:
+    obs = np.ascontiguousarray(obs, np.int32)
+    S, T = obs.shape
+    N = hmm.nstates()
+    rows = np.empty((S, T, N), np.float32)
+    mu, r = np.empty((S, T), np.float32), np.empty((S, T), np.float32)
+    E, path = np.empty(S, np.float32), np.empty((S, T), np.int32)
+    ptr = lambda x: x.ctypes.data_as(ctypes.c_void_p)
+    L.check(L.lib().cv_f32ru_trace(hmm.handle, S, T, ptr(obs), ptr(rows), ptr(mu), ptr(r), ptr(E), ptr(path)))
+    return dict(rows=rows.transpose(1, 0, 2), mu=mu, r=r, E=E, path=path)
+
+
 def device_memory() -> dict:
     cur, peak = ctypes.c_int64(), ctypes.c_int64()
     L.check(L.lib().cv_device_memory(ctypes.byref(cur), ctypes.byref(peak)))
diff --git a/include/cviterbi.h b/include/cviterbi.h
--- a/include/cviterbi.h
+++ b/include/cviterbi.h
@@ -117,6 +117,9 @@
                                         uint8_t* status_dev);
 CV_API int32_t cv_last_t64_stats(const cv_hmm* h, int64_t* out, int32_t n);
 CV_API int32_t cv_last_fixed_first_stats(const cv_hmm* h, int64_t* out, int32_t n);
+CV_API int32_t cv_last_first_pass_kind(const cv_hmm* h);
+CV_API cv_status cv_f32ru_trace(cv_hmm* h, int64_t nseq, int64_t T, const int32_t* obs, float* rows, float* mu,
+                                float* r, float* e_last, int32_t* path);
 CV_API cv_status cv_last_timing(cv_hmm* h, cv_timing* out);
 CV_API cv_status cv_timing_begin(cv_hmm* h);
 CV_API cv_status cv_timing_end(cv_hmm* h, cv_timing* out);
```

After: 80.97 billion, median of 6. +7.5%, better.
